# aurelienpierreeng/ansel

Hardware: AMD Instinct MI355X
Metric: MPix/s full export pixelpipe (100 MP raw); % MI355X HBM roofline (higher is better)
Workload: dtype f32

## Files before the change

### ansel_amd/csrc/denoiseprofile.hip

```cpp
#define ANSEL_MATH_DEFAULT_TABS tabs_lds
#include "hip_common.h"
#include "pipe_fused.h"
#include "rgb_chain_kernel.h"
#include "devmath.h"
#include "nlmeans_core_params.h"

#include <math.h>
#include <utility>

using namespace ansel;

namespace
{

#define BANDS DT_HIP_DENOISEPROFILE_BANDS
#define P_FULCRUM 0.05f

__host__ __device__ __forceinline__ float max_first(const float a, const float b) { return a > b ? a : b; }
__host__ __device__ __forceinline__ float min_first(const float a, const float b) { return a < b ? a : b; }
__device__ __forceinline__ int clampi(const int v, const int lo, const int hi) { return v < lo ? lo : (v > hi ? hi : v); }

struct dn_setup
{
  int max_scale;
// ... 248 lines not shown
  const float k0 = fmaf(x, 1056964608.0f - 1065353216.0f, 1065353216.0f);
  return __int_as_float(k0 >= 8388608.0f ? (int)k0 : 0);
}

__device__ __forceinline__ float mexp2_of_clamped(const float arg)
{
  const float k0 = fmaf(arg, 1056964608.0f - 1065353216.0f, 1065353216.0f);
  int k;
  asm("v_cvt_i32_f32 %0, %1" : "=v"(k) : "v"(k0));
  k = min(k, 0x3f800000);
  return __int_as_float(k >= 0x800000 ? k : 0);
}

__device__ __forceinline__ int walk_row(const int b, const int height, const int mult)
{
  if(height <= mult) return b < height ? b : -1;
  const int per_pass = (height + mult - 1) / mult;
  const int row = (b % per_pass) * mult + b / per_pass;
  return row < height ? row : -1;
}

__device__ __forceinline__ double wave_sum_halving(double v)
{
#pragma unroll
  for(int off = 32; off >= 1; off >>= 1) v += __shfl_down(v, off, 64);
  return v;
}

#ifdef ANSEL_HIP_MEASURING
__global__ __launch_bounds__(256) void dn_decompose(const float4 *__restrict__ in, float4 *__restrict__ coarse,
                                                    float4 *__restrict__ detail, double *__restrict__ partial,
                                                    const int width, const int height, const int mult,
                                                    const float inv_sigma2, const int nseg, const int in_row0,
                                                    const int in_rows)
{
  __shared__ double runs[4][4];
  const int bx = xcd_col();
  if(bx >= nseg) return;
  const int row = walk_row(blockIdx.y, height, mult);
  if(row < 0) return;
  const int col = bx * 256 + threadIdx.x;
  double sq[4] = { 0.0, 0.0, 0.0, 0.0 };
  if(col < width)
  {
    const float4 px = in[(size_t)(row + in_row0) * width + col];
    float sum[4] = { 0.f, 0.f, 0.f, 0.f }, wgt = 0.f;
#pragma unroll
    for(int jj = 0; jj < 5; jj++)
    {
      const size_t y = (size_t)clampi(row + in_row0 + mult * (jj - 2), 0, in_rows - 1) * width;
      const float fj = jj == 0 || jj == 4 ? 0.0625f : (jj == 2 ? 0.375f : 0.25f);
#pragma unroll
      for(int ii = 0; ii < 5; ii++)
      {
        const int x = clampi(col + mult * (ii - 2), 0, width - 1);
        const float fi = ii == 0 || ii == 4 ? 0.0625f : (ii == 2 ? 0.375f : 0.25f);
        const float4 p2 = in[y + x];
        const float dx = px.x - p2.x, dy = px.y - p2.y, dz = px.z - p2.z;
        const float dot = (dx * dx + dy * dy + dz * dz) * inv_sigma2;
        const float arg = dot * 0.02f - 9.0f;
        const float wp = mexp2_of_clamped(arg);
        const float w = (fi * fj) * wp;
        wgt += w;
        sum[0] += w * p2.x;
        sum[1] += w * p2.y;
        sum[2] += w * p2.z;
        sum[3] += w * p2.w;
      }
    }
    float c4[4], d4[4];
    const float pin[4] = { px.x, px.y, px.z, px.w };
#pragma unroll
    for(int c = 0; c < 4; c++)
    {
      c4[c] = sum[c] / wgt;
      d4[c] = pin[c] - c4[c];
      sq[c] = (double)(d4[c] * d4[c]);
    }
    const size_t o = (size_t)row * width + col;
    coarse[o] = make_float4(c4[0], c4[1], c4[2], c4[3]);
    if(detail) detail[o] = make_float4(d4[0], d4[1], d4[2], d4[3]);
  }
  const int wave = threadIdx.x >> 6, lane = threadIdx.x & 63;
#pragma unroll
  for(int c = 0; c < 4; c++)
  {
    const double s = wave_sum_halving(sq[c]);
    if(lane == 0) runs[wave][c] = s;
  }
  __syncthreads();
  if(threadIdx.x < 4)
  {
    const int c = threadIdx.x;
    const double seg = ((runs[0][c] + runs[1][c]) + runs[2][c]) + runs[3][c];
    partial[4 * ((size_t)row * nseg + bx) + c] = seg;
  }
}
#endif

#define DN_RING 6
__device__ __forceinline__ float dn_photometric(const float4 px, const float4 p2, const float inv_sigma2)
{
  const float dx = px.x - p2.x, dy = px.y - p2.y, dz = px.z - p2.z;
  const float dot = (dx * dx + dy * dy + dz * dz) * inv_sigma2;
  const float arg = dot * 0.02f - 9.0f;
  return mexp2_of_clamped(arg);
}
__device__ __forceinline__ double wave_sum4_halving(const double q0, const double q1, const double q2, const double q3)
{
  union d2
  {
    double d;
    unsigned u[2];
  };
  auto level = [](const double a, const double b, const bool rows16) {
    d2 x, y, rx, ry;
    x.d = a;
    y.d = b;
#pragma unroll
    for(int h = 0; h < 2; h++)
    {
      const auto r = rows16 ? __builtin_amdgcn_permlane16_swap(x.u[h], y.u[h], false, false)
                            : __builtin_amdgcn_permlane32_swap(x.u[h], y.u[h], false, false);
      rx.u[h] = r[0];
      ry.u[h] = r[1];
    }
    return rx.d + ry.d;
  };
  const double s01 = level(q0, q1, false), s23 = level(q2, q3, false);
  d2 t;
  t.d = level(s01, s23, true);
#define DN_ROW_SHL(n)                                                                                     \
  {                                                                                                       \
    d2 o;                                                                                                 \
    o.u[0] = (unsigned)__builtin_amdgcn_update_dpp(0, (int)t.u[0], 0x100 + (n), 0xf, 0xf, true);          \
    o.u[1] = (unsigned)__builtin_amdgcn_update_dpp(0, (int)t.u[1], 0x100 + (n), 0xf, 0xf, true);          \
    t.d = t.d + o.d;                                                                                      \
  }
  DN_ROW_SHL(8)
  DN_ROW_SHL(4)
  DN_ROW_SHL(2)
  DN_ROW_SHL(1)
#undef DN_ROW_SHL
  return t.d;
}

struct dn_strip_kernargs
{
  const float4 *in;
  float4 *coarse, *detail;
  double *partial;
  int width, height, mult_arg;
  float inv_sigma2;
  int nseg, in_row0, in_rows, strip, strips_per_class;
  vst_args fa;
  unsigned *alpha_flag;
  int flag_sense;
};
template <bool PRE, int MULT, bool ALPHA0> constexpr int dn_strip_waves()
{
  if(PRE && MULT == 0) return 6;
  const int lds = DN_RING * (256 + 4 * (MULT ? MULT : 1)) * (ALPHA0 ? 12 : 16);
  const int wgs = (160 * 1024) / lds;
  return wgs >= 8 ? 8 : (wgs < 1 ? 1 : wgs);
}
template <bool PRE, int MULT, bool ALPHA0, bool P3 = false>
__global__ __launch_bounds__(256) __attribute__((amdgpu_waves_per_eu(dn_strip_waves<PRE, MULT, ALPHA0>(), 8))) void dn_decompose_strip(const float4 *__restrict__ in, float4 *__restrict__ coarse,
                                                          float4 *__restrict__ detail, double *__restrict__ partial,
                                                          const int width, const int height, const int mult_arg,
                                                          const float inv_sigma2, const int nseg, const int in_row0,
                                                          const int in_rows, const int strip, const int strips_per_class,
                                                          const vst_args fa_by_value, unsigned *__restrict__ alpha_flag, const int flag_sense)
{
  const vst_args &fa = kernarg_at<vst_args>((int)offsetof(dn_strip_kernargs, fa));
  (void)fa_by_value;
  if(PRE) ansel_math::stage_default_tables(threadIdx.x);
  if(flag_sense == 1 && *alpha_flag) return;
  if(flag_sense == 2 && !*alpha_flag) return;
  unsigned alpha_bits = 0;
  const int mult = MULT ? MULT : mult_arg;
  constexpr bool LATE2 = PRE && MULT == 1;
  const bool have_t3 = PRE && fa.vst == 2;
  const float t3_of_zero = have_t3 ? dn_vst_y0u0v0_alpha(0.0f, fa) : 0.0f;
#define DN_FETCH(p) (PRE ? dn_precondition_pixel((p), fa, t3_of_zero, have_t3) : (p))
  static_assert(!P3 || ALPHA0, "three-float planes are the ALPHA0 launches'");
  auto in_at = [&](const size_t i) -> float4 {
    if(P3 && !PRE)
    {
      const float *const p3 = reinterpret_cast<const float *>(in) + 3 * i;
      return make_float4(p3[0], p3[1], p3[2], 0.0f);
    }
    return in[i];
  };
  auto plane_put = [&](float4 *const plane, const size_t i, const float v0, const float v1, const float v2, const float v3) {
    if(P3)
    {
      float *const p3 = reinterpret_cast<float *>(plane) + 3 * i;
      p3[0] = v0;
      p3[1] = v1;
      p3[2] = v2;
    }
    else
      plane[i] = make_float4(v0, v1, v2, v3);
  };
  __shared__ double runs[2][4][4];
  const int bx = blockIdx.x;
  const int cls = blockIdx.y / strips_per_class, k0 = (blockIdx.y - cls * strips_per_class) * strip;
  const int n_cls = (height - cls + mult - 1) / mult;
  if(k0 >= n_cls) return;
  const int nrows = min(strip, n_cls - k0);
  const int r_first = cls + k0 * mult;
  const int tw = 256 + 4 * mult;
  extern __shared__ float4 ring[];
  float *const ringf = reinterpret_cast<float *>(ring);
  auto ring_put = [&](const int slot, const int c, const float4 v) {
    if(ALPHA0)
    {
      ringf[(slot * 3 + 0) * tw + c] = v.x;
      ringf[(slot * 3 + 1) * tw + c] = v.y;
      ringf[(slot * 3 + 2) * tw + c] = v.z;
    }
    else
      ring[slot * tw + c] = v;
  };
  auto ring_get = [&](const int slot, const int c) -> float4 {
    if(ALPHA0) return make_float4(ringf[(slot * 3 + 0) * tw + c], ringf[(slot * 3 + 1) * tw + c], ringf[(slot * 3 + 2) * tw + c], 0.0f);
    return ring[slot * tw + c];
  };
  const int tid = threadIdx.x, wave = tid >> 6, lane = tid & 63;
  const int col = bx * 256 + tid;
  const int ecol0 = clampi(bx * 256 - 2 * mult + tid, 0, width - 1), ecol1 = clampi(bx * 256 - 2 * mult + tid + 256, 0, width - 1);
  const bool second = tid + 256 < tw;
#define DN_IN_ROW(q) ((size_t)clampi(r_first + ((q) - 2) * mult + in_row0, 0, in_rows - 1) * width)
#pragma unroll
  for(int q = 0; q < 4; q++)
  {
    const size_t y = DN_IN_ROW(q);
    ring_put(q, tid, DN_FETCH(in_at(y + ecol0)));
    if(second) ring_put(q, tid + 256, DN_FETCH(in_at(y + ecol1)));
  }
  float4 n0, n1 = make_float4(0.f, 0.f, 0.f, 0.f);
  {
    const size_t y = DN_IN_ROW(4);
    n0 = in_at(y + ecol0);
    if(!LATE2 && second) n1 = in_at(y + ecol1);
  }
  int s0 = 0;
  float up1 = 0.f, up2 = 0.f, up2_next = 0.f;
  __syncthreads();
  {
    const float4 c0 = ring_get(2, tid + 2 * mult), c1 = ring_get(3, tid + 2 * mult);
    const float4 a0 = ring_get(0, tid + 2 * mult), a1 = ring_get(1, tid + 2 * mult);
    up2 = dn_photometric(c0, a0, inv_sigma2);
    up1 = dn_photometric(c0, a1, inv_sigma2);
    up2_next = dn_photometric(c1, a1, inv_sigma2);
  }
  for(int k = 0; k < nrows; k++)
  {
    {
      const int sl = s0 + 4 >= DN_RING ? s0 + 4 - DN_RING : s0 + 4;
      ring_put(sl, tid, DN_FETCH(n0));
      if(LATE2) { if(second) ring_put(sl, tid + 256, DN_FETCH(in_at(DN_IN_ROW(k + 4) + ecol1))); }
      else if(second) ring_put(sl, tid + 256, DN_FETCH(n1));
    }
    __syncthreads();
    if(k > 0 && tid < 4)
    {
      const int c = tid, pr = (k - 1) & 1;
      const double seg = ((runs[pr][0][c] + runs[pr][1][c]) + runs[pr][2][c]) + runs[pr][3][c];
      partial[4 * ((size_t)(r_first + (k - 1) * mult) * nseg + bx) + c] = seg;
    }
    if(k + 1 < nrows)
    {
      const size_t y = DN_IN_ROW(k + 5);
      n0 = in_at(y + ecol0);
      if(!LATE2 && second) n1 = in_at(y + ecol1);
    }
    const int row = r_first + k * mult;
    double sq[4] = { 0.0, 0.0, 0.0, 0.0 };
    if(col < width)
    {
      const int sc = s0 + 2 >= DN_RING ? s0 + 2 - DN_RING : s0 + 2;
      const float4 px = ring_get(sc, tid + 2 * mult);
      float sum[4] = { 0.f, 0.f, 0.f, 0.f }, wgt = 0.f, down1 = 0.f, down2 = 0.f;
#pragma unroll
      for(int jj = 0; jj < 5; jj++)
      {
        const int sl = s0 + jj >= DN_RING ? s0 + jj - DN_RING : s0 + jj;
        const float fj = jj == 0 || jj == 4 ? 0.0625f : (jj == 2 ? 0.375f : 0.25f);
        float4 tap[5];
#pragma unroll
        for(int ii = 0; ii < 5; ii++) tap[ii] = ring_get(sl, tid + ii * mult);
#pragma unroll
        for(int ii = 0; ii < 5; ii++)
        {
          const float fi = ii == 0 || ii == 4 ? 0.0625f : (ii == 2 ? 0.375f : 0.25f);
          const float4 p2 = tap[ii];
          float wp;
          if(ii == 2 && jj == 0) wp = up2;
          else if(ii == 2 && jj == 1) wp = up1;
          else wp = dn_photometric(px, p2, inv_sigma2);
          if(ii == 2 && jj == 3) down1 = wp;
          if(ii == 2 && jj == 4) down2 = wp;
          const float w = (fi * fj) * wp;
          wgt += w;
          sum[0] += w * p2.x;
          sum[1] += w * p2.y;
          sum[2] += w * p2.z;
          if(!ALPHA0) sum[3] += w * p2.w;
        }
        asm volatile("" : "+v"(wgt), "+v"(sum[0]), "+v"(sum[1]), "+v"(sum[2]), "+v"(sum[3]) : : "memory");
      }
      up1 = down1;
      up2 = up2_next;
      up2_next = down2;
      float c4[4], d4[4];
      const float pin[4] = { px.x, px.y, px.z, px.w };
#pragma unroll
      for(int c = 0; c < 4; c++)
      {
        if(ALPHA0 && c == 3)
        {
          c4[3] = __builtin_amdgcn_ballot_w64(!(wgt > 0.0f)) == 0ull ? 0.0f : 0.0f / wgt;
          alpha_bits |= __float_as_uint(c4[3]);
        }
        else
          c4[c] = sum[c] / wgt;
        d4[c] = pin[c] - c4[c];
        sq[c] = (double)(d4[c] * d4[c]);
      }
      const size_t o = (size_t)row * width + col;
      plane_put(coarse, o, c4[0], c4[1], c4[2], c4[3]);
      if(detail) plane_put(detail, o, d4[0], d4[1], d4[2], d4[3]);
    }
    {
      const double s = wave_sum4_halving(sq[0], sq[1], sq[2], sq[3]);
      if((lane & 15) == 0) runs[k & 1][wave][((lane >> 5) & 1) | ((lane >> 3) & 2)] = s;
    }
    s0 = s0 + 1 == DN_RING ? 0 : s0 + 1;
  }
#undef DN_IN_ROW
#undef DN_FETCH
  __syncthreads();
  if(tid < 4)
  {
    const int c = tid, pr = (nrows - 1) & 1;
    const double seg = ((runs[pr][0][c] + runs[pr][1][c]) + runs[pr][2][c]) + runs[pr][3][c];
    partial[4 * ((size_t)(r_first + (nrows - 1) * mult) * nseg + bx) + c] = seg;
  }
  if(ALPHA0 && alpha_flag && __builtin_amdgcn_ballot_w64(alpha_bits != 0) != 0ull && lane == 0) atomicOr(alpha_flag, 1u);
}

static void launch_decompose(hipStream_t st, const float4 *in, float4 *coarse, float4 *detail, double *partial, const int width,
                             const int height, const int mult, const float inv_sigma2, const int nseg, const int in_row0,
                             const int in_rows, const vst_args *pre = nullptr, unsigned *alpha_flag = nullptr, const int mode = 0)
{
#ifdef ANSEL_HIP_MEASURING
  static const bool per_row = getenv("ANSEL_HIP_DN_PER_ROW") != nullptr;
  if(per_row && !pre)
  {
    const int rows = (height <= mult) ? height : ((height + mult - 1) / mult) * mult;
    dn_decompose<<<dim3(xcd_pad(nseg), rows), 256, 0, st>>>(in, coarse, detail, partial, width, height, mult, inv_sigma2, nseg,
                                                            in_row0, in_rows);
    return;
  }
#endif
  const int classes = height < mult ? height : mult, per_class = (height + mult - 1) / mult;
  const int strip = strip_rows(nseg, classes, per_class);
  const int strips_per_class = (per_class + strip - 1) / strip;
  const dim3 grid(nseg, classes * strips_per_class);
  size_t lds = (size_t)DN_RING * (256 + 4 * mult) * sizeof(float);
#ifdef ANSEL_HIP_MEASURING
  static const char *const pad_env = measuring_env("ANSEL_HIP_DN_LDS_PAD");
  const size_t lds_pad = pad_env ? (size_t)atoi(pad_env) : 0;
#else
  const size_t lds_pad = 0;
#endif
#define DN_LDS(A0_) (lds * ((A0_) ? 3 : 4) + lds_pad)
  vst_args none;
  memset(&none, 0, sizeof(none));
#define DN_LAUNCH_(PRE_, M_, A0_, FA_, SENSE_)                                                                                          \
  dn_decompose_strip<PRE_, M_, A0_><<<grid, 256, DN_LDS(A0_), st>>>(in, coarse, detail, partial, width, height, mult, inv_sigma2, nseg, in_row0, \
                                                            in_rows, strip, strips_per_class, FA_, alpha_flag, SENSE_)
#define DN_LAUNCH(PRE_, M_, FA_)                  \
  do                                              \
  {                                               \
    if(mode == 1)                                 \
      dn_decompose_strip<PRE_, M_, true, true><<<grid, 256, DN_LDS(true), st>>>(in, coarse, detail, partial, width, height, mult, inv_sigma2, nseg, in_row0, \
                                                            in_rows, strip, strips_per_class, FA_, alpha_flag, 0); \
    else if(mode == 2)                            \
      DN_LAUNCH_(PRE_, M_, false, FA_, 2);        \
    else if(alpha_flag && (PRE_))                 \
      DN_LAUNCH_(PRE_, M_, true, FA_, 0);         \
    else if(alpha_flag)                           \
    {                                             \
      DN_LAUNCH_(PRE_, M_, true, FA_, 1);         \
      DN_LAUNCH_(PRE_, M_, false, FA_, 2);        \
    }                                             \
    else                                          \
      DN_LAUNCH_(PRE_, M_, false, FA_, 0);        \
  } while(0)
  if(pre)
  {
    if(mult == 1) DN_LAUNCH(true, 1, *pre);
    else DN_LAUNCH(true, 0, *pre);
  }
  else
    switch(mult)
    {
      case 1: DN_LAUNCH(false, 1, none); break;
      case 2: DN_LAUNCH(false, 2, none); break;
      case 4: DN_LAUNCH(false, 4, none); break;
      case 8: DN_LAUNCH(false, 8, none); break;
      case 16: DN_LAUNCH(false, 16, none); break;
      case 32: DN_LAUNCH(false, 32, none); break;
      case 64: DN_LAUNCH(false, 64, none); break;
      default: DN_LAUNCH(false, 0, none); break;
    }
#undef DN_LAUNCH
#undef DN_LAUNCH_
#undef DN_LDS
}

struct thr_args
{
  size_t n_partial;
  float n1;
  float sb2;
  float adjt[4];
};

#define THR_GROUPS 16
__global__ __launch_bounds__(64) void dn_band_sums(const double *__restrict__ partial_all, const size_t n_partial,
                                                  double *__restrict__ acc_all )
{
  const double *const partial = partial_all + (size_t)blockIdx.y * n_partial * 4;
  double *const acc = acc_all + (size_t)blockIdx.y * 4 * 1024;
  const int t = blockIdx.x * 64 + threadIdx.x;
  double s[4] = { 0.0, 0.0, 0.0, 0.0 };
  typedef double d4 __attribute__((ext_vector_type(4)));
  const d4 *const p4 = (const d4 *)partial;
  size_t k = t;
  for(; k + 7 * 1024 < n_partial; k += 8 * 1024)
  {
    d4 v[8];
#pragma unroll
    for(int u = 0; u < 8; u++) v[u] = p4[k + (size_t)u * 1024];
#pragma unroll
    for(int u = 0; u < 8; u++)
    {
      s[0] += v[u].x;
      s[1] += v[u].y;
      s[2] += v[u].z;
      s[3] += v[u].w;
    }
  }
  for(; k < n_partial; k += 1024)
  {
    const d4 v = p4[k];
    s[0] += v.x;
    s[1] += v.y;
    s[2] += v.z;
    s[3] += v.w;
  }
#pragma unroll
  for(int c = 0; c < 4; c++) acc[c * 1024 + t] = s[c];
}

struct thr_args_all
{
  thr_args band[BANDS];
};
__global__ __launch_bounds__(1024) void dn_band_threshold(const double *__restrict__ sums_all ,
                                                          const thr_args_all all, float *__restrict__ thrs_all)
{
  __shared__ double acc[4][1024];
  const double *const sums = sums_all + (size_t)blockIdx.x * 4 * 1024;
  const thr_args &a = all.band[blockIdx.x];
  float *const thrs = thrs_all + 4 * blockIdx.x;
  const int t = threadIdx.x;
#pragma unroll
  for(int c = 0; c < 4; c++) acc[c][t] = sums[c * 1024 + t];
  __syncthreads();
  for(int off = 512; off >= 1; off >>= 1)
  {
    if(t < off)
    {
#pragma unroll
      for(int c = 0; c < 4; c++) acc[c][t] += acc[c][t + off];
    }
    __syncthreads();
  }
  if(t < 4)
  {
    const float sum_y2 = (float)acc[t][0];
    const float std_x = t < 3 ? sqrtf(max_first(1e-6f, sum_y2 / a.n1 - a.sb2)) : 1.0f;
    thrs[t] = a.adjt[t] * a.sb2 / std_x;
  }
}


bool invert3(const float in[3][4], float out[3][4])
{
  const float A = in[1][1] * in[2][2] - in[1][2] * in[2][1];
  const float B = -in[1][0] * in[2][2] + in[1][2] * in[2][0];
  const float C = in[1][0] * in[2][1] - in[1][1] * in[2][0];
  const float D = -in[0][1] * in[2][2] + in[0][2] * in[2][1];
  const float E = in[0][0] * in[2][2] - in[0][2] * in[2][0];
  const float F = -in[0][0] * in[2][1] + in[0][1] * in[2][0];
  const float G = in[0][1] * in[1][2] - in[0][2] * in[1][1];
  const float H = -in[0][0] * in[1][2] + in[0][2] * in[1][0];
  const float I = in[0][0] * in[1][1] - in[0][1] * in[1][0];
  const float det = in[0][0] * A + in[0][1] * B + in[0][2] * C;
  if(det == 0.0f) return false;
  const float r = 1.0f / det;
  out[0][0] = r * A; out[0][1] = r * D; out[0][2] = r * G; out[0][3] = 0.0f;
  out[1][0] = r * B; out[1][1] = r * E; out[1][2] = r * H; out[1][3] = 0.0f;
  out[2][0] = r * C; out[2][1] = r * F; out[2][2] = r * I; out[2][3] = 0.0f;
  return true;
}

void setup(const dt_hip_piece_t *piece, const dt_hip_denoiseprofile_data_t *d, dn_setup &s, const bool nlm)
{
  memset(&s, 0, sizeof(s));
  const float in_scale = fminf((float)piece->roi_in.scale, 1.0f);
  const float big = (float)(piece->roi_in.height > piece->roi_in.width ? piece->roi_in.height : piece->roi_in.width);
  const float supp0 = min_first((float)(2 * (2u << (BANDS - 1)) + 1), big * 0.2f);
  const float i0 = log2f((supp0 - 1.0f) * .5f);
  int max_scale = 0;
  for(; max_scale < BANDS; max_scale++)
  {
    const float supp = (float)(2 * (2u << max_scale) + 1);
    const float supp_in = supp * (1.0f / in_scale);
    const float i_in = log2f((supp_in - 1) * .5f) - 1.0f;
    const float t = 1.0f - (i_in + .5f) / i0;
    if(t < 0.0f) break;
  }
  s.max_scale = max_scale;

  const float weights[4] = { nlm ? 1.0f : 2.0f, 1.0f, nlm ? 1.0f : 2.0f, 0.0f };
  const float wb_mean = (d->wb_coeffs[0] + d->wb_coeffs[1] + d->wb_coeffs[2]) / 3.0f;
  float *wb = s.wb;
// ... 216 lines not shown
    synth_args none;
    memset(&none, 0, sizeof(none));
    dn_finish<<<pixel_grid(npix_out), 256, 0, st>>>((float4 *)dev_out, nullptr, npix_out, ia, none);
  }
  return check_launch("dn_finish");
}

int wavelets_runnable(const dt_hip_piece_t *piece, const dn_setup &s)
{
  const int w = piece->roi_in.width, h = piece->roi_in.height;
  if(s.max_scale < 1)
  {
    set_last_error("denoiseprofile: frame too small for a single wavelet band");
    return -1;
  }
  const int max_mult = 1 << (s.max_scale - 1);
  if(w < 2 * max_mult || h < 2 * max_mult) return 0;
  if(w < 4 * max_mult)
  {
    set_last_error("denoiseprofile: %d columns is less than 4x the coarsest dilation %d", w, max_mult);
    return -1;
  }
  return 1;
}

}

namespace ansel
{

struct dn_band_job_t
{
  int devid, w, frame_h, max_scale, row0, rows;
  dt_hip_denoiseprofile_data_t d;
  dn_setup s;
  dev_buf_t cur;
  int cur_top, cur_bottom;
  dev_buf_t det[BANDS];
  dev_buf_t sums;
  dev_buf_t local;
  dev_buf_t thrs;
  int next_scale;
  bool sums_requested;
};

void denoiseprofile_band_abort(dn_band_job_t *j)
{
  delete j;
}

int denoiseprofile_halo_rows(const dt_hip_piece_t *piece, const dt_hip_denoiseprofile_data_t *d)
{
  if(DT_HIP_DENOISEPROFILE_IS_NLMEANS(d->mode)) return nlmeans_core_halo_rows(piece->roi_in.height, nlm_params_of(piece, d));
  dn_setup s;
  setup(piece, d, s, false);
  if(wavelets_runnable(piece, s) != 1) return -1;
  return 2;
}

static int clip_halo(const int h, const int avail) { return h < avail ? h : avail; }

int denoiseprofile_band_begin(int devid, const dt_hip_piece_t *piece, const dt_hip_denoiseprofile_data_t *d,
                              const band_view_t *band, const int buf_rows, dt_hip_mem_t dev_in, dt_hip_mem_t dev_out,
                              dn_band_job_t **job)
{
  *job = nullptr;
  if(!valid_device(devid) || !piece || !d || !band || !dev_in || buf_rows <= 0) return DT_HIP_INVALID_ARG;
  if(piece->channels != 4 || !(piece->roi_in.scale > 0.0)) return DT_HIP_INVALID_ARG;
  if(DT_HIP_DENOISEPROFILE_IS_NLMEANS(d->mode)) return denoise_nlmeans(devid, piece, d, band, buf_rows, dev_in, dev_out);
  if(!DT_HIP_DENOISEPROFILE_IS_WAVELETS(d->mode)) return DT_HIP_INVALID_ARG;
  dn_band_job_t *j = new dn_band_job_t();
  j->devid = devid;
  j->w = piece->roi_in.width;
  j->frame_h = band->frame_h;
  j->row0 = band->row0;
  j->rows = band->row1 - band->row0;
  j->d = *d;
  setup(piece, d, j->s, false);
  if(wavelets_runnable(piece, j->s) != 1)
  {
    delete j;
    return DT_HIP_INVALID_ARG;
  }
  j->max_scale = j->s.max_scale;
  const int w = j->w, nseg = (w + 255) / 256;
  const size_t npix = (size_t)w * buf_rows;
  const size_t n_frame = (size_t)band->frame_h * nseg;
  const size_t sums_bytes = (size_t)j->max_scale * n_frame * 4 * sizeof(double);
  j->cur_top = band->row0 - band->buf_row0;
  j->cur_bottom = buf_rows - j->cur_top - j->rows;
  bool ok = (bool)(j->cur = dev_buf_t::alloc(devid, npix * sizeof(float4)));
  ok &= (bool)(j->sums = dev_buf_t::alloc(devid, sums_bytes));
  ok &= (bool)(j->local = dev_buf_t::alloc(devid, (size_t)j->rows * nseg * 4 * sizeof(double)));
  ok &= (bool)(j->thrs = dev_buf_t::alloc(devid, BANDS * 4 * sizeof(float)));
  if(!ok || j->cur_bottom < 0)
  {
    denoiseprofile_band_abort(j);
    return DT_HIP_SYSMEM_ALLOCATION;
  }
  hipStream_t st = stream_of(devid);
  if(hipMemsetAsync(j->sums.ptr(), 0, sums_bytes, st) != hipSuccess)
  {
    denoiseprofile_band_abort(j);
    return DT_HIP_DEFAULT_ERROR;
  }
  {
    vst_args fa;
    forward_args(j->s, fa);
    launch_scope ls(devid, "dn_precondition");
    dn_precondition<<<pixel_grid(npix), 256, 0, st>>>((const float4 *)dev_in, j->cur.as<float4>(), npix, fa);
  }
  const int err = check_launch("dn_precondition");
  if(err != DT_HIP_SUCCESS)
  {
    denoiseprofile_band_abort(j);
    return err;
  }
  *job = j;
  return DT_HIP_SUCCESS;
}

int denoiseprofile_band_step(dn_band_job_t *j, dt_hip_mem_t *halo_buf, int *halo_rows, double **sums, size_t *sum_count)
{
  *halo_buf = nullptr;
  *halo_rows = 0;
  *sums = nullptr;
  *sum_count = 0;
  const int devid = j->devid, w = j->w, nseg = (w + 255) / 256;
  const size_t n_frame = (size_t)j->frame_h * nseg;
  if(j->next_scale >= j->max_scale)
  {
    if(j->sums_requested) return 0;
    j->sums_requested = true;
    *sums = j->sums.as<double>();
    *sum_count = (size_t)j->max_scale * n_frame * 4;
    return 2;
  }
  hipStream_t st = stream_of(devid);
  const int scale = j->next_scale, mult = 1 << scale;
  const bool last = scale + 1 == j->max_scale;
  const int h_next = last ? 0 : 2 * (2 << scale);
  const int top = clip_halo(h_next, j->row0), bottom = clip_halo(h_next, j->frame_h - j->row0 - j->rows);
  dev_buf_t coarse = dev_buf_t::alloc(devid, (size_t)(top + j->rows + bottom) * w * sizeof(float4));
  j->det[scale] = dev_buf_t::alloc(devid, (size_t)j->rows * w * sizeof(float4));
  if(!coarse || !j->det[scale])
  {
    denoiseprofile_band_abort(j);
    return DT_HIP_SYSMEM_ALLOCATION;
  }
  const float varf = sqrtf(2.0f + 2.0f * 4.0f * 4.0f + 6.0f * 6.0f) / 16.0f;
  const float sigma_band = powf(varf, scale) * 1.0f;
  {
    launch_scope ls(devid, "dn_decompose");
    launch_decompose(st, j->cur.as<float4>(), coarse.as<float4>() + (size_t)top * w, j->det[scale].as<float4>(), j->local.as<double>(), w, j->rows, mult,
                     1.0f / (sigma_band * sigma_band), nseg, j->cur_top, j->cur_top + j->rows + j->cur_bottom);
  }
  int err = check_launch("denoiseprofile band decompose");
  if(err == DT_HIP_SUCCESS
     && hipMemcpyAsync(j->sums.as<double>() + ((size_t)scale * n_frame + (size_t)j->row0 * nseg) * 4, j->local.ptr(),
                       (size_t)j->rows * nseg * 4 * sizeof(double), hipMemcpyDeviceToDevice, st) != hipSuccess)
    err = DT_HIP_DEFAULT_ERROR;
  j->cur = std::move(coarse);
  j->cur_top = top;
  j->cur_bottom = bottom;
  j->next_scale++;
  if(err != DT_HIP_SUCCESS)
  {
    denoiseprofile_band_abort(j);
    return err;
  }
  if(!last && (top || bottom))
  {
    *halo_buf = j->cur.ptr();
    *halo_rows = h_next;
    return 1;
  }
  return denoiseprofile_band_step(j, halo_buf, halo_rows, sums, sum_count);
}

int denoiseprofile_band_finish(dn_band_job_t *j, dt_hip_mem_t dev_out)
{
  if(!j || !dev_out) return DT_HIP_INVALID_ARG;
  const int devid = j->devid, nseg = (j->w + 255) / 256;
  const size_t npix = (size_t)j->w * j->rows, n_frame = (size_t)j->frame_h * nseg;
  hipStream_t st = stream_of(devid);
  float4 *out = (float4 *)dev_out;
  int err = DT_HIP_SUCCESS;
  synth_args sy;
  memset(&sy, 0, sizeof(sy));
  sy.nbands = j->max_scale;
  sy.thrs = j->thrs.as<float>();
  const dev_buf_t accs_buf = dev_buf_t::alloc(devid, (size_t)BANDS * 4 * 1024 * sizeof(double));
  double *const accs = accs_buf.as<double>();
  if(!accs) err = DT_HIP_SYSMEM_ALLOCATION;
  thr_args_all all;
  memset(&all, 0, sizeof(all));
  for(int scale = 0; scale < j->max_scale; scale++)
  {
    all.band[scale].n_partial = n_frame;
    threshold_args(&j->d, scale, j->max_scale, (size_t)j->w * j->frame_h, all.band[scale]);
    sy.detail[scale] = j->det[scale].as<float4>();
  }
  if(err == DT_HIP_SUCCESS)
  {
    launch_scope ls(devid, "dn_band_threshold");
    dn_band_sums<<<dim3(THR_GROUPS, j->max_scale), 64, 0, st>>>(j->sums.as<double>(), n_frame, accs);
    dn_band_threshold<<<j->max_scale, 1024, 0, st>>>(accs, all, j->thrs.as<float>());
    err = check_launch("denoiseprofile band threshold");
  }
  if(err == DT_HIP_SUCCESS)
  {
    vst_args ia;
    inverse_args(j->s, ia);
    launch_scope ls(devid, "dn_finish");
    dn_finish<<<pixel_grid(npix), 256, 0, st>>>(out, j->cur.as<float4>() + (size_t)j->cur_top * j->w, npix, ia, sy);
    err = check_launch("dn_finish");
  }
  denoiseprofile_band_abort(j);
  return err;
}

}

extern "C" {

static int denoiseprofile_run(int devid, const dt_hip_piece_t *piece, const dt_hip_denoiseprofile_data_t *d, dt_hip_mem_t dev_in,
                              dt_hip_mem_t dev_out, const rgb_group_t *chain)
{
  if(!valid_device(devid) || !piece || !d || !dev_in || !dev_out) return DT_HIP_INVALID_ARG;
  if(!DT_HIP_DENOISEPROFILE_IS_WAVELETS(d->mode) && !DT_HIP_DENOISEPROFILE_IS_NLMEANS(d->mode))
  {
    set_last_error("denoiseprofile: mode %d is not implemented on device (wavelets and non-local means are)", d->mode);
    return DT_HIP_INVALID_ARG;
  }
  if(piece->channels != 4 || !(piece->roi_in.scale > 0.0)) return DT_HIP_INVALID_ARG;
  const int w = piece->roi_in.width, h = piece->roi_in.height;
  if(w <= 0 || h <= 0) return DT_HIP_SUCCESS;
  const size_t npix = (size_t)w * h, plane = npix * sizeof(float4);
  if(DT_HIP_DENOISEPROFILE_IS_NLMEANS(d->mode))
    return chain ? DT_HIP_INVALID_ARG : denoise_nlmeans(devid, piece, d, nullptr, h, dev_in, dev_out);
  chain_args ca;
  int cm_kind = CM_NONE, fm = FM_NONE;
  if(chain)
  {
    if(chain->pre_lab || chain->to_u16 || chain->width != w || chain->height != h) return DT_HIP_INVALID_ARG;
    if(rgb_group_fill_args(*chain, ca, cm_kind, fm) != DT_HIP_SUCCESS || fm != FM_NONE) return DT_HIP_INVALID_ARG;
  }
  dn_setup s;
  setup(piece, d, s, false);
  const int runnable = wavelets_runnable(piece, s);
  if(runnable < 0) return DT_HIP_INVALID_ARG;
  hipStream_t st = stream_of(devid);
  if(!runnable) return chain ? DT_HIP_INVALID_ARG : dt_hip_enqueue_copy_buffer_to_buffer(devid, dev_in, dev_out, 0, 0, plane);
  const int nseg = (w + 255) / 256;
  const size_t n_partial = (size_t)h * nseg;
  const dev_buf_t partial_buf = dev_buf_t::alloc(devid, (size_t)BANDS * n_partial * 4 * sizeof(double));
  const dev_buf_t thrs_buf = dev_buf_t::alloc(devid, BANDS * 4 * sizeof(float));
  const dev_buf_t accs_buf = dev_buf_t::alloc(devid, (size_t)BANDS * 4 * 1024 * sizeof(double));
  double *const partial = partial_buf.as<double>(), *const accs = accs_buf.as<double>();
  float *const thrs = thrs_buf.as<float>();
  int err = (partial && thrs && accs) ? DT_HIP_SUCCESS : DT_HIP_SYSMEM_ALLOCATION;
  synth_args sy;
  memset(&sy, 0, sizeof(sy));
  sy.nbands = s.max_scale;
  sy.thrs = thrs;
  dev_buf_t coarse_buf[BANDS];
  float4 *coarse[BANDS] = { nullptr };
  const dev_buf_t det0_buf = dev_buf_t::alloc(devid, plane);
  float4 *const det0 = det0_buf.as<float4>();
  if(!det0) err = DT_HIP_SYSMEM_ALLOCATION;
  for(int k = 0; k < s.max_scale && err == DT_HIP_SUCCESS; k++)
  {
    coarse[k] = (coarse_buf[k] = dev_buf_t::alloc(devid, plane)).as<float4>();
    if(!coarse[k]) err = DT_HIP_SYSMEM_ALLOCATION;
    sy.detail[k] = k == 0 ? det0 : coarse[k];
  }
  sy.coarse0 = coarse[0];
  float4 *out = (float4 *)dev_out;
  vst_args fa;
  forward_args(s, fa);
  const float4 *b1 = (const float4 *)dev_in;
  dev_buf_t alpha_buf;
  unsigned *alpha_flag = nullptr;
  if(err == DT_HIP_SUCCESS && s.vst == 2)
  {
    alpha_flag = (alpha_buf = dev_buf_t::alloc(devid, sizeof(unsigned))).as<unsigned>();
    if(!alpha_flag) err = DT_HIP_SYSMEM_ALLOCATION;
    else if(hipMemsetAsync(alpha_flag, 0, sizeof(unsigned), st) != hipSuccess) err = DT_HIP_DEFAULT_ERROR;
  }
  const int sequences = alpha_flag ? 2 : 1;
  for(int seq = 0; seq < sequences && err == DT_HIP_SUCCESS; seq++)
  {
    b1 = (const float4 *)dev_in;
    for(int scale = 0; scale < s.max_scale && err == DT_HIP_SUCCESS; scale++)
    {
      const int mult = 1 << scale;
      const float varf = sqrtf(2.0f + 2.0f * 4.0f * 4.0f + 6.0f * 6.0f) / 16.0f;
      const float sigma_band = powf(varf, scale) * 1.0f;
      {
        launch_scope ls(devid, "dn_decompose");
        launch_decompose(st, b1, coarse[scale], scale == 0 ? det0 : nullptr, partial + (size_t)scale * n_partial * 4, w, h, mult,
                         1.0f / (sigma_band * sigma_band), nseg, 0, h, scale == 0 ? &fa : nullptr, alpha_flag, alpha_flag ? seq + 1 : 0);
      }
      err = check_launch("denoiseprofile band");
      b1 = coarse[scale];
    }
  }
  if(err == DT_HIP_SUCCESS)
  {
    thr_args_all all;
    memset(&all, 0, sizeof(all));
    for(int scale = 0; scale < s.max_scale; scale++)
    {
      all.band[scale].n_partial = n_partial;
      threshold_args(d, scale, s.max_scale, npix, all.band[scale]);
    }
    launch_scope ls(devid, "dn_band_threshold");
    dn_band_sums<<<dim3(THR_GROUPS, s.max_scale), 64, 0, st>>>(partial, n_partial, accs);
    dn_band_threshold<<<s.max_scale, 1024, 0, st>>>(accs, all, thrs);
    err = check_launch("denoiseprofile thresholds");
  }
  if(err == DT_HIP_SUCCESS)
  {
    vst_args ia;
    inverse_args(s, ia);
    const unsigned grid = pixel_grid(npix);
    for(int seq = 0; seq < sequences; seq++)
    {
      launch_scope ls(devid, chain ? "dn_finish_chain" : "dn_finish");
      if(alpha_flag)
      {
        sy.planes3 = seq == 0;
        sy.gate = alpha_flag;
        sy.gate_sense = seq + 1;
      }
      if(!chain) dn_finish<<<grid, 256, 0, st>>>(out, b1, npix, ia, sy);
      else
        switch(cm_kind)
        {
          case CM_NONE: dn_finish_chain<CM_NONE><<<grid, 256, 0, st>>>(out, b1, npix, ia, sy, ca); break;
          case 0: dn_finish_chain<0><<<grid, 256, 0, st>>>(out, b1, npix, ia, sy, ca); break;
          case 1: dn_finish_chain<1><<<grid, 256, 0, st>>>(out, b1, npix, ia, sy, ca); break;
          case 2: dn_finish_chain<2><<<grid, 256, 0, st>>>(out, b1, npix, ia, sy, ca); break;
          case 3: dn_finish_chain<3><<<grid, 256, 0, st>>>(out, b1, npix, ia, sy, ca); break;
          default: dn_finish_chain<4><<<grid, 256, 0, st>>>(out, b1, npix, ia, sy, ca); break;
        }
    }
    err = check_launch("dn_finish");
  }
  return err;
}

int dt_hip_iop_denoiseprofile_process(int devid, const dt_hip_piece_t *piece, const dt_hip_denoiseprofile_data_t *d,
                                      dt_hip_mem_t dev_in, dt_hip_mem_t dev_out)
{
  return denoiseprofile_run(devid, piece, d, dev_in, dev_out, nullptr);
}
}

namespace ansel
{
int denoiseprofile_process_chain(int devid, const dt_hip_piece_t *piece, const dt_hip_denoiseprofile_data_t *d,
                                 dt_hip_mem_t dev_in, dt_hip_mem_t dev_out, const rgb_group_t *chain)
{
  if(!chain) return DT_HIP_INVALID_ARG;
  return denoiseprofile_run(devid, piece, d, dev_in, dev_out, chain);
}
}

extern "C" {


void dt_hip_iop_denoiseprofile_tiling(const dt_hip_piece_t *piece, const dt_hip_denoiseprofile_data_t *d,
                                      dt_hip_tiling_t *tiling)
{
  memset(tiling, 0, sizeof(*tiling));
  tiling->maxbuf = tiling->maxbuf_cl = 1.0f;
  tiling->xalign = tiling->yalign = 1;
  if(DT_HIP_DENOISEPROFILE_IS_NLMEANS(d->mode))
  {
    const float scale = fminf(fminf((float)piece->roi_in.scale, 2.0f), 1.0f);
    const int P = (int)ceilf(d->radius * scale), K = (int)ceilf(d->nbhood * scale);
    const int K_scattered = (int)ceilf(d->scattering * (K * K * K + 7.0 * K * sqrt((double)K)) / 6.0) + K;
    tiling->factor = 2.0f + 0.25f;
    tiling->factor_cl = 3.0f;
    tiling->overlap = (unsigned)(P + K_scattered);
  }
  else
  {
    dn_setup s;
    setup(piece, d, s, false);
    tiling->factor = 5.0f;
    tiling->factor_cl = 3.0f + (float)s.max_scale + 1.0f / 64.0f;
    tiling->overlap = 1u << s.max_scale;
  }
}

}
```

### ansel_amd/csrc/diffuse.hip

```cpp
#include "hip_common.h"

#include <type_traits>
#include "devmath.h"
#include "ieee_inrange.h"
#include "px_colorspaces.h"

#include <math.h>
#include <cstdlib>

namespace ansel
{
int bspline_launch_decompose(int devid, hipStream_t s, const float4 *in, float4 *hf, float4 *lf, int w, int h, int mult,
                             const unsigned *gate = nullptr);
int bspline_launch_decompose3(int devid, hipStream_t s, const void *in, bool in4, float *lf, int w, int h, int mult, unsigned *alpha_flag);
#ifdef ANSEL_HIP_MEASURING
int bspline_launch_decompose2(int devid, hipStream_t s, const float4 *in, float4 *low1, float4 *low2, int w, int h, int mult);
#endif
}
using namespace ansel;

namespace
{

#define DIFFUSE_MAX_SCALES 10
// ... 250 lines not shown
      H4[3 * ii + jj] = hf[rows[ii] + cols[jj]];
      L4[3 * ii + jj] = lf[rows[ii] + cols[jj]];
    }
  const int tw = 256 + 2 * a.mult;
  const int tx = threadIdx.x;
  float4 energy = make_float4(0.f, 0.f, 0.f, 0.f);
  if(SHARED)
  {
#pragma unroll
    for(int ii = 0; ii < 3; ii++)
    {
      const float4 h = H4[3 * ii + 1], l = L4[3 * ii + 1];
      r2s[ii * tw + tx + a.mult] = make_float4(ratio2(h.x, l.x), ratio2(h.y, l.y), ratio2(h.z, l.z), ratio2(h.w, l.w));
    }
    if(tx < a.mult)
    {
#pragma unroll
      for(int ii = 0; ii < 3; ii++)
      {
        const float4 h = H4[3 * ii], l = L4[3 * ii];
        r2s[ii * tw + tx] = make_float4(ratio2(h.x, l.x), ratio2(h.y, l.y), ratio2(h.z, l.z), ratio2(h.w, l.w));
      }
    }
    if(tx >= 256 - a.mult)
    {
#pragma unroll
      for(int ii = 0; ii < 3; ii++)
      {
        const float4 h = H4[3 * ii + 2], l = L4[3 * ii + 2];
        r2s[ii * tw + tx + 2 * a.mult] = make_float4(ratio2(h.x, l.x), ratio2(h.y, l.y), ratio2(h.z, l.z), ratio2(h.w, l.w));
      }
    }
    __syncthreads();
    if(col >= a.width) return;
#pragma unroll
    for(int ii = 0; ii < 3; ii++)
    {
#pragma unroll
      for(int jj = 0; jj < 3; jj++)
      {
        const float4 r = r2s[ii * tw + tx + jj * a.mult];
        energy.x += r.x;
        energy.y += r.y;
        energy.z += r.z;
        energy.w += r.w;
      }
      asm volatile("" : "+v"(energy.x), "+v"(energy.y), "+v"(energy.z), "+v"(energy.w) : : "memory");
    }
  }
  else
  {
    if(col >= a.width) return;
#pragma unroll
    for(int k = 0; k < 9; k++)
    {
      energy.x += ratio2(H4[k].x, L4[k].x);
      energy.y += ratio2(H4[k].y, L4[k].y);
      energy.z += ratio2(H4[k].z, L4[k].z);
      energy.w += ratio2(H4[k].w, L4[k].w);
    }
  }
  if(mask && !mask[(size_t)row * a.width + col])
  {
    const size_t c = (size_t)row * a.width + col;
    const float4 h = H4[4], l = L4[4];
    const float4 o = make_float4(max_zero(h.x + l.x), max_zero(h.y + l.y), max_zero(h.z + l.z), max_zero(h.w + l.w));
    if(final_pass) nt_store(out + c, o);
    else out[c] = o;
    return;
  }
  float H[9], L[9];
  float4 o;
#pragma unroll
  for(int k = 0; k < 9; k++) { H[k] = H4[k].x; L[k] = L4[k].x; }
  o.x = pde_channel(H, L, energy.x, a);
#pragma unroll
  for(int k = 0; k < 9; k++) { H[k] = H4[k].y; L[k] = L4[k].y; }
  o.y = pde_channel(H, L, energy.y, a);
#pragma unroll
  for(int k = 0; k < 9; k++) { H[k] = H4[k].z; L[k] = L4[k].z; }
  o.z = pde_channel(H, L, energy.z, a);
  if(alpha_is_blank(H4, L4))
    o.w = 0.0f;
  else
  {
#pragma unroll
    for(int k = 0; k < 9; k++) { H[k] = H4[k].w; L[k] = L4[k].w; }
    o.w = pde_channel(H, L, energy.w, a);
  }
  const size_t idx = rows[1] + col;
  if(final_pass) nt_store(out + idx, o);
  else out[idx] = o;
}

#define PDE_RING 4
#define PDE_DMA_MAX_MULT 16
#if defined(__HIP_DEVICE_COMPILE__) && !defined(__gfx950__)
#error "pde_dma_planes(): LDS-DMA of 16 bytes per lane and its hazard padding are written for gfx950 only"
#endif
template <int NPL>
__device__ __forceinline__ void pde_dma_planes(const float4 *const p0, const float4 *const p1, const float4 *const p2, const unsigned voff,
                                               const unsigned d0, const unsigned d1, const unsigned d2)
{
  unsigned keep;
  if constexpr(NPL == 3)
    asm volatile("s_waitcnt lgkmcnt(0)\n\ts_nop 4\n\ts_mov_b32 %0, m0\n\t"
                 "s_mov_b32 m0, %5\n\ts_nop 0\n\tglobal_load_lds_dwordx4 %1, %2\n\t"
                 "s_mov_b32 m0, %6\n\ts_nop 0\n\tglobal_load_lds_dwordx4 %1, %3\n\t"
                 "s_mov_b32 m0, %7\n\ts_nop 0\n\tglobal_load_lds_dwordx4 %1, %4\n\t"
                 "s_mov_b32 m0, %0"
                 : "=&s"(keep)
                 : "v"(voff), "s"(p0), "s"(p1), "s"(p2), "s"(d0), "s"(d1), "s"(d2)
                 : "memory");
  else
    asm volatile("s_waitcnt lgkmcnt(0)\n\ts_nop 4\n\ts_mov_b32 %0, m0\n\t"
                 "s_mov_b32 m0, %4\n\ts_nop 0\n\tglobal_load_lds_dwordx4 %1, %2\n\t"
                 "s_mov_b32 m0, %5\n\ts_nop 0\n\tglobal_load_lds_dwordx4 %1, %3\n\t"
                 "s_mov_b32 m0, %0"
                 : "=&s"(keep)
                 : "v"(voff), "s"(p0), "s"(p2), "s"(d0), "s"(d2)
                 : "memory");
}
template <bool H0_4>
__device__ __forceinline__ void pde_dma_planes3(const void *const p0, const void *const p1, const void *const p2, const unsigned voff0,
                                                const unsigned voff, const unsigned d0, const unsigned d1, const unsigned d2)
{
  unsigned keep;
  if constexpr(H0_4)
    asm volatile("s_waitcnt lgkmcnt(0)\n\ts_nop 4\n\ts_mov_b32 %0, m0\n\t"
                 "s_mov_b32 m0, %6\n\ts_nop 0\n\tglobal_load_lds_dwordx4 %1, %3\n\t"
                 "s_mov_b32 m0, %7\n\ts_nop 0\n\tglobal_load_lds_dwordx3 %2, %4\n\t"
                 "s_mov_b32 m0, %8\n\ts_nop 0\n\tglobal_load_lds_dwordx3 %2, %5\n\t"
                 "s_mov_b32 m0, %0"
                 : "=&s"(keep)
                 : "v"(voff0), "v"(voff), "s"(p0), "s"(p1), "s"(p2), "s"(d0), "s"(d1), "s"(d2)
                 : "memory");
  else
    asm volatile("s_waitcnt lgkmcnt(0)\n\ts_nop 4\n\ts_mov_b32 %0, m0\n\t"
                 "s_mov_b32 m0, %5\n\ts_nop 0\n\tglobal_load_lds_dwordx3 %1, %2\n\t"
                 "s_mov_b32 m0, %6\n\ts_nop 0\n\tglobal_load_lds_dwordx3 %1, %3\n\t"
                 "s_mov_b32 m0, %7\n\ts_nop 0\n\tglobal_load_lds_dwordx3 %1, %4\n\t"
                 "s_mov_b32 m0, %0"
                 : "=&s"(keep)
                 : "v"(voff), "s"(p0), "s"(p1), "s"(p2), "s"(d0), "s"(d1), "s"(d2)
                 : "memory");
}
struct pde_px3
{
  float x, y, z;
};
template <bool HSUB, int MODE, bool DMA, int L3>
__device__ __forceinline__ void pde_strip_body(const float4 *__restrict__ hf, const float4 *__restrict__ hsub,
                                               const float4 *__restrict__ lf, float4 *__restrict__ out, const pde_args &a,
                                               const int final_pass, const unsigned char *__restrict__ mask, const int strip,
                                               const int strips_per_class)
{
  static_assert(L3 == 0 || (HSUB && DMA), "three-float planes: the low-pass chain's LDS-DMA form only");
  if(a.gate && ((*a.gate != 0u) == (a.gate_sense == 1))) return;
  extern __shared__ float4 r2s[];
  pde_px3 *const r2s3 = reinterpret_cast<pde_px3 *>(r2s);
  const int mult = a.mult;
  const int cls = blockIdx.y / strips_per_class, k0s = (blockIdx.y - cls * strips_per_class) * strip;
  const int n_cls = (a.height - cls + mult - 1) / mult;
  if(k0s >= n_cls) return;
  const int nrows = (strip < n_cls - k0s) ? strip : n_cls - k0s;
  const int r_first = cls + k0s * mult;
  const int tx = threadIdx.x, tw = 256 + 2 * mult;
  const int col = (int)blockIdx.x * 256 + tx;
  const bool live = col < a.width;
  const int cols[3] = { clampi(col - mult, 0, a.width - 1), clampi(col, 0, a.width - 1), clampi(col + mult, 0, a.width - 1) };
#define PDE_ROW(v) ((size_t)clampi(r_first + ((v) - 1) * mult, 0, a.height - 1) * a.width)
  float4 Hw[3][3], Lw[3][3];
  constexpr int NPL = HSUB ? 3 : 2;
  const int lane = tx & 63, zw = 64 + 2 * mult;
  float4 *const zone = r2s + PDE_RING * tw + (tx >> 6) * NPL * zw;
  float4 *const zone3 = reinterpret_cast<float4 *>(reinterpret_cast<char *>(r2s) + (size_t)PDE_RING * tw * 12) + (tx >> 6) * 3 * zw;
  using lds_f4_ptr = __attribute__((address_space(3))) float4 *;
  const unsigned zone_lds = !DMA ? 0u : (unsigned)__builtin_amdgcn_readfirstlane((int)(unsigned)(__UINTPTR_TYPE__)(lds_f4_ptr)(
                                           L3 ? zone3 : zone));
  const unsigned off_main = (unsigned)cols[0] * 16u, off_halo = (unsigned)clampi(col - mult + 64, 0, a.width - 1) * 16u;
  auto dma_row = [&](const int v) {
    const size_t y = PDE_ROW(v);
    if constexpr(L3 != 0)
    {
      const unsigned m3 = (unsigned)cols[0] * 12u, h3 = (unsigned)clampi(col - mult + 64, 0, a.width - 1) * 12u;
      const unsigned p0 = (unsigned)zw * 16u, p1 = 2u * p0;
      const void *const b0 = L3 == 2 ? (const void *)(hf + y) : (const void *)((const float *)hf + 3 * y);
      const void *const b1 = (const float *)hsub + 3 * y, *const b2 = (const float *)lf + 3 * y;
      pde_dma_planes3<L3 == 2>(b0, b1, b2, L3 == 2 ? off_main : m3, m3, zone_lds, zone_lds + p0, zone_lds + p1);
      if(lane < 2 * mult)
        pde_dma_planes3<L3 == 2>(b0, b1, b2, L3 == 2 ? off_halo : h3, h3, zone_lds + 1024u, zone_lds + p0 + 1024u, zone_lds + p1 + 1024u);
      return;
    }
    const unsigned pl = (unsigned)zw * 16u;
    pde_dma_planes<NPL>(hf + y, hsub + y, lf + y, off_main, zone_lds, zone_lds + pl, zone_lds + (NPL - 1) * pl);
    if(lane < 2 * mult)
      pde_dma_planes<NPL>(hf + y, hsub + y, lf + y, off_halo, zone_lds + 1024u, zone_lds + pl + 1024u, zone_lds + (NPL - 1) * pl + 1024u);
  };
  struct
  {
    float4 o;
    size_t idx;
    bool have;
  } pending;
  pending.have = false;
  auto store = [&](const size_t i, const float4 o) {
    if(final_pass) nt_store(out + i, o);
    else if constexpr(L3 != 0)
    {
      float *const p3 = (float *)out + 3 * i;
      p3[0] = o.x;
      p3[1] = o.y;
      p3[2] = o.z;
    }
    else out[i] = o;
  };
  auto fetch_row = [&](const int v, auto slot_tag) {
    constexpr int SL = decltype(slot_tag)::value;
    const size_t y = PDE_ROW(v);
    float4 c[3], low[3];
    if constexpr(DMA)
    {
      asm volatile("s_waitcnt vmcnt(0)" : : : "memory");
      if constexpr(L3 != 0)
      {
#pragma unroll
        for(int jj = 0; jj < 3; jj++)
        {
          const int x = lane + jj * mult;
          const float4 v0 = zone3[x], v1 = zone3[zw + x], v2 = zone3[2 * zw + x];
          c[jj] = make_float4(v0.x, v0.y, v0.z, 0.0f);
          low[jj] = make_float4(v1.x, v1.y, v1.z, 0.0f);
          Lw[SL][jj] = make_float4(v2.x, v2.y, v2.z, 0.0f);
        }
      }
      else
#pragma unroll
      for(int jj = 0; jj < 3; jj++)
      {
        c[jj] = zone[lane + jj * mult];
        if(HSUB) low[jj] = zone[zw + lane + jj * mult];
        Lw[SL][jj] = zone[(NPL - 1) * zw + lane + jj * mult];
      }
    }
    else if(PDE_OFF(a, 2) && v >= 2)
    {
#pragma unroll
      for(int jj = 0; jj < 3; jj++)
      {
        c[jj] = Hw[SL][jj];
        low[jj] = make_float4(0.f, 0.f, 0.f, 0.f);
      }
    }
    else
    {
#pragma unroll
      for(int jj = 0; jj < 3; jj++)
      {
        c[jj] = hf[y + cols[jj]];
        if(HSUB) low[jj] = hsub[y + cols[jj]];
        Lw[SL][jj] = lf[y + cols[jj]];
      }
    }
    __builtin_amdgcn_sched_barrier(0);
#pragma unroll
    for(int jj = 0; jj < 3; jj++)
      Hw[SL][jj] = HSUB ? make_float4(c[jj].x - low[jj].x, c[jj].y - low[jj].y, c[jj].z - low[jj].z, c[jj].w - low[jj].w) : c[jj];
    float4 *const ring = r2s + (v % PDE_RING) * tw;
    auto ratios = [&](const float4 h, const float4 l) {
      const bool blank = a.wskip && __builtin_amdgcn_ballot_w64((__float_as_uint(h.w) | __float_as_uint(l.w)) != 0) == 0ull;
      return ratio2_rgb(h, l, blank ? 0.0f : ratio2(h.w, l.w), PDE_APPROX(a));
    };
    if(PDE_OFF(a, 4)) return;
    if constexpr(L3 != 0)
    {
      pde_px3 *const ring3 = r2s3 + (v % PDE_RING) * tw;
      auto put = [&](const int x, const float4 h, const float4 l) {
        const float4 r = ratio2_rgb(h, l, 0.0f, PDE_APPROX(a));
        ring3[x] = { r.x, r.y, r.z };
      };
      put(tx + mult, Hw[SL][1], Lw[SL][1]);
      if(tx < mult) put(tx, Hw[SL][0], Lw[SL][0]);
      if(tx >= 256 - mult) put(tx + 2 * mult, Hw[SL][2], Lw[SL][2]);
      return;
    }
    ring[tx + mult] = ratios(Hw[SL][1], Lw[SL][1]);
    if(tx < mult) ring[tx] = ratios(Hw[SL][0], Lw[SL][0]);
    if(tx >= 256 - mult) ring[tx + 2 * mult] = ratios(Hw[SL][2], Lw[SL][2]);
  };
  auto row_step = [&](auto t_tag, const int kk) {
    constexpr int T = decltype(t_tag)::value, S0 = T, S1 = (T + 1) % 3, S2 = (T + 2) % 3;
    constexpr bool WIDE_READS = MODE >= 0 && !(((MODE % 3) | ((MODE / 9) % 3)) && (((MODE / 3) % 3) | ((MODE / 27) % 3)));
    fetch_row(kk + 2, std::integral_constant<int, S2>());
    if constexpr(DMA)
    {
      if(pending.have)
      {
        store(pending.idx, pending.o);
        pending.have = false;
      }
      if(kk + 1 < nrows) dma_row(kk + 3);
    }
    if(!PDE_OFF(a, 1)) __syncthreads();
    if(!live) return;
    const float4 H4[9] = { Hw[S0][0], Hw[S0][1], Hw[S0][2], Hw[S1][0], Hw[S1][1], Hw[S1][2], Hw[S2][0], Hw[S2][1], Hw[S2][2] };
    const float4 L4[9] = { Lw[S0][0], Lw[S0][1], Lw[S0][2], Lw[S1][0], Lw[S1][1], Lw[S1][2], Lw[S2][0], Lw[S2][1], Lw[S2][2] };
    const int row = r_first + kk * mult;
    const bool blank = L3 != 0 || alpha_is_blank(H4, L4);
    __builtin_amdgcn_sched_barrier(0);
    if(pending.have && !PDE_OFF(a, 8))
    {
      store(pending.idx, pending.o);
      pending.have = false;
    }
    __builtin_amdgcn_sched_barrier(0);
    float4 energy = make_float4(0.f, 0.f, 0.f, 0.f);
    if(PDE_OFF(a, 4)) energy = make_float4(0.5f, 0.5f, 0.5f, 0.5f);
    else if constexpr(L3 != 0)
#pragma unroll
    for(int ii = 0; ii < 3; ii++)
    {
      const pde_px3 *const ring = r2s3 + ((kk + ii) % PDE_RING) * tw + tx;
#pragma unroll
      for(int jj = 0; jj < 3; jj++)
      {
        const pde_px3 r = ring[jj * mult];
        energy.x += r.x;
        energy.y += r.y;
        energy.z += r.z;
      }
      if(!WIDE_READS || ii >= 1) asm volatile("" : "+v"(energy.x), "+v"(energy.y), "+v"(energy.z) : : "memory");
    }
    else
#pragma unroll
    for(int ii = 0; ii < 3; ii++)
    {
      const float4 *const ring = r2s + ((kk + ii) % PDE_RING) * tw + tx;
#pragma unroll
      for(int jj = 0; jj < 3; jj++)
      {
        const float4 r = ring[jj * mult];
        energy.x += r.x;
        energy.y += r.y;
        energy.z += r.z;
        if(!(blank && a.wskip)) energy.w += r.w;
      }
      if(!WIDE_READS || ii >= 1) asm volatile("" : "+v"(energy.x), "+v"(energy.y), "+v"(energy.z), "+v"(energy.w) : : "memory");
    }
    const size_t idx = (size_t)row * a.width + col;
    float4 o;
    if(L3 == 0 && mask && !mask[idx])
    {
      const float4 h = H4[4], l = L4[4];
      o = make_float4(max_zero(h.x + l.x), max_zero(h.y + l.y), max_zero(h.z + l.z), max_zero(h.w + l.w));
    }
    else if(PDE_OFF(a, 16))
      o = make_float4(H4[4].x + energy.x, L4[4].y + energy.y, H4[0].z + energy.z, L4[8].w);
    else
    {
      float H[9], L[9];
#pragma unroll
      for(int k = 0; k < 9; k++) { H[k] = H4[k].x; L[k] = L4[k].x; }
      o.x = pde_channel<MODE>(H, L, energy.x, a);
#pragma unroll
      for(int k = 0; k < 9; k++) { H[k] = H4[k].y; L[k] = L4[k].y; }
      o.y = pde_channel<MODE>(H, L, energy.y, a);
#pragma unroll
      for(int k = 0; k < 9; k++) { H[k] = H4[k].z; L[k] = L4[k].z; }
      o.z = pde_channel<MODE>(H, L, energy.z, a);
      if(blank)
        o.w = 0.0f;
      else
      {
#pragma unroll
        for(int k = 0; k < 9; k++) { H[k] = H4[k].w; L[k] = L4[k].w; }
        o.w = pde_channel<MODE>(H, L, energy.w, a);
      }
    }
    if(a.post_lab) o = px_rgb_to_lab(o, a.post_m);
    pending.o = o;
    pending.idx = idx;
    pending.have = true;
  };
  if constexpr(DMA) dma_row(0);
  fetch_row(0, std::integral_constant<int, 0>());
  if constexpr(DMA) dma_row(1);
  fetch_row(1, std::integral_constant<int, 1>());
  if constexpr(DMA) dma_row(2);
  for(int kk = 0; kk < nrows; kk += 3)
  {
    row_step(std::integral_constant<int, 0>(), kk);
    if(kk + 1 < nrows) row_step(std::integral_constant<int, 1>(), kk + 1);
    if(kk + 2 < nrows) row_step(std::integral_constant<int, 2>(), kk + 2);
  }
  if constexpr(DMA) asm volatile("s_waitcnt vmcnt(0)" : : : "memory");
  if(pending.have) store(pending.idx, pending.o);
#undef PDE_ROW
}

template <bool HSUB, int MODE, bool DMA = false>
__global__ __launch_bounds__(256, 3) void diffuse_pde_strip(const float4 *__restrict__ hf, const float4 *__restrict__ hsub,
                                                         const float4 *__restrict__ lf,
                                                         float4 *__restrict__ out, const pde_args a, const int final_pass,
                                                         const unsigned char *__restrict__ mask, const int strip,
                                                         const int strips_per_class)
{
  pde_strip_body<HSUB, MODE, DMA, 0>(hf, hsub, lf, out, a, final_pass, mask, strip, strips_per_class);
}
template <int MODE, bool H0_4>
__global__ __launch_bounds__(256, 3) void diffuse_pde_strip3(const float4 *__restrict__ hf, const float4 *__restrict__ hsub,
                                                          const float4 *__restrict__ lf, float4 *__restrict__ out, const pde_args a,
                                                          const int final_pass, const int strip, const int strips_per_class)
{
  pde_strip_body<true, MODE, true, H0_4 ? 2 : 1>(hf, hsub, lf, out, a, final_pass, nullptr, strip, strips_per_class);
}

__device__ __forceinline__ uint32_t splitmix32(const uint64_t seed)
{
  uint64_t result = (seed ^ (seed >> 33)) * 0x62a9d9ed799705f5ull;
  result = (result ^ (result >> 28)) * 0xcb24d0a5c88c35b3ull;
  return (uint32_t)(result >> 32);
}

__device__ __forceinline__ float xoshiro128plus(uint32_t state[4])
{
  const uint32_t result = state[0] + state[3];
  const uint32_t t = state[1] << 9;
  state[2] ^= state[0];
  state[3] ^= state[1];
  state[1] ^= state[2];
  state[0] ^= state[3];
  state[2] ^= t;
  state[3] = (state[3] << 11) | (state[3] >> 21);
  return (float)(result >> 8) * 0x1.0p-24f;
}

__device__ __forceinline__ float gaussian_noise(const float mu, const float sigma, const bool flip, uint32_t state[4])
{
  const float x1 = xoshiro128plus(state);
  const float u1 = x1 > 1.17549435e-38f ? x1 : 1.17549435e-38f;
  const float u2 = xoshiro128plus(state);
  const float angle = (float)(6.283185307179586 * (double)u2);
  const float radius = sqrtf(-2.0f * ansel_math::logf_exact(u1));
  const float noise = flip ? radius * ansel_math::cosf_exact(angle) : radius * ansel_math::sinf_exact(angle);
  return noise * sigma + mu;
}

__global__ __launch_bounds__(256) void diffuse_inpaint(const float4 *__restrict__ in, float4 *__restrict__ out,
                                                       unsigned char *__restrict__ mask, const float threshold,
                                                       const size_t npixels, const size_t width, const size_t first_pixel)
{
  const size_t p = (size_t)blockIdx.x * blockDim.x + threadIdx.x;
  if(p >= npixels) return;
  const float4 v = in[p];
  const bool m = v.x > threshold || v.y > threshold || v.z > threshold;
  mask[p] = m ? 1 : 0;
  float4 o = v;
  if(m)
  {
    const size_t k = 4 * (p + first_pixel);
    const uint32_t i = (uint32_t)(k / width);
    const uint32_t j = (uint32_t)(k - i);
    uint32_t state[4] = { splitmix32((uint32_t)(j + 1)), splitmix32((uint64_t)(uint32_t)(j + 1) * (uint32_t)(i + 3)),
                          splitmix32(1337), splitmix32(666) };
    xoshiro128plus(state);
    xoshiro128plus(state);
    xoshiro128plus(state);
    xoshiro128plus(state);
    const bool flip = (i % 2) || (j % 2);
    o.x = fabsf(gaussian_noise(v.x, v.x, flip, state));
    o.y = fabsf(gaussian_noise(v.y, v.y, flip, state));
    o.z = fabsf(gaussian_noise(v.z, v.z, flip, state));
    o.w = fabsf(gaussian_noise(v.w, v.w, flip, state));
  }
  out[p] = o;
}

inline float sqf(const float x) { return x * x; }

float sigma_at_step(const float sigma, const unsigned s)
{
  float acc = sigma;
  for(unsigned k = 1; k <= s; k++) acc = sqrtf(sqf(acc) + sqf(exp2f((float)k) * sigma));
  return acc;
}

unsigned steps_to_sigma(const float sigma_filter, const float sigma_final)
{
  unsigned s = 0;
  float radius = sigma_filter;
  while(radius < sigma_final)
  {
    ++s;
    radius = sqrtf(sqf(radius) + sqf((float)(1 << s) * sigma_filter));
  }
  return s + 1;
}

int scales_of(const dt_hip_piece_t *piece, const dt_hip_diffuse_data_t *d)
{
  const float zoom = (float)(d->iscale / piece->roi_in.scale);
  const float final_radius = (float)(d->radius + d->radius_center) * 2.0f / zoom;
  const int s = (int)steps_to_sigma(BSPLINE_SIGMA, final_radius);
  return s < 1 ? 1 : (s > DIFFUSE_MAX_SCALES ? DIFFUSE_MAX_SCALES : s);
}

}

namespace ansel
{
int diffuse_halo_rows(const dt_hip_piece_t *piece, const dt_hip_diffuse_data_t *d)
{
  if(!(d->iscale > 0.0f) || !(piece->roi_in.scale > 0.0)) return -1;
  const int scales = scales_of(piece, d);
  const int it_req = (int)ceilf((float)d->iterations);
  const int iterations = it_req > 1 ? it_req : 1;
  return iterations * 3 * ((1 << scales) - 1);
}
}

extern "C" {

int dt_hip_iop_diffuse_process(int devid, const dt_hip_piece_t *piece, const dt_hip_diffuse_data_t *d,
                               dt_hip_mem_t dev_in, dt_hip_mem_t dev_out)
{
  return diffuse_process_rows(devid, piece, d, 0, dev_in, dev_out);
}

}

namespace ansel
{
static void *g_diffuse_probe = nullptr;

static int diffuse_run(int devid, const dt_hip_piece_t *piece, const dt_hip_diffuse_data_t *d, int first_row, dt_hip_mem_t dev_in,
                       dt_hip_mem_t dev_out, const dt_hip_lab_data_t *post_lab);
int diffuse_process_rows(int devid, const dt_hip_piece_t *piece, const dt_hip_diffuse_data_t *d, int first_row,
                         dt_hip_mem_t dev_in, dt_hip_mem_t dev_out)
{
  return diffuse_run(devid, piece, d, first_row, dev_in, dev_out, nullptr);
}
int diffuse_process_post_lab(int devid, const dt_hip_piece_t *piece, const dt_hip_diffuse_data_t *d, dt_hip_mem_t dev_in,
                             dt_hip_mem_t dev_out, const dt_hip_lab_data_t *lab)
{
  if(!lab || measuring_env("ANSEL_HIP_PDE_PER_ROW")) return DT_HIP_INVALID_ARG;
  return diffuse_run(devid, piece, d, 0, dev_in, dev_out, lab);
}

struct diffuse_planes_t
{
  dev_buf_t hf[DIFFUSE_MAX_SCALES], lf[2], tmp[2];
  dev_buf_t mask;
  dev_buf_t inpainted;
  dev_buf_t alpha_flag;
};

struct diffuse_job_t
{
  int devid;
  hipStream_t st;
  const dt_hip_diffuse_data_t *d;
  const dt_hip_lab_data_t *post_lab;
  int w, h, scales, iterations;
  float zoom;
  bool lf_chain;
  bool per_row, no_dma;
  diffuse_planes_t p;
};

static int diffuse_alloc_planes(diffuse_job_t &j, const bool in_place, const bool three)
{
  diffuse_planes_t &p = j.p;
  const size_t plane = (size_t)j.w * j.h * sizeof(float4);
  bool ok = true;
  for(int s = 0; s < j.scales; s++) ok &= (bool)(p.hf[s] = dev_buf_t::alloc(j.devid, plane));
  for(int k = 0; k < ((j.lf_chain && !in_place) ? 1 : 2); k++) ok &= (bool)(p.lf[k] = dev_buf_t::alloc(j.devid, plane));
  for(int k = 0; k < 2 && k < j.iterations - 1; k++) ok &= (bool)(p.tmp[k] = dev_buf_t::alloc(j.devid, plane));
  if(ok && three) ok &= (bool)(p.alpha_flag = dev_buf_t::alloc(j.devid, sizeof(unsigned)));
  if(ok && j.d->threshold > 0.0f)
  {
    p.mask = dev_buf_t::alloc(j.devid, (size_t)j.w * j.h);
    if(!p.tmp[1]) p.tmp[1] = dev_buf_t::alloc(j.devid, plane);
    p.inpainted = dev_buf_t::borrow(p.tmp[1].base());
    ok = p.mask && p.inpainted;
  }
  return ok ? DT_HIP_SUCCESS : DT_HIP_SYSMEM_ALLOCATION;
}

static void pde_args_of_call(pde_args &a, const int w, const int h, const dt_hip_diffuse_data_t *d)
{
  memset(&a, 0, sizeof(a));
  a.width = w;
  a.height = h;
  a.wskip = measuring_env("ANSEL_HIP_PDE_NO_WSKIP") ? 0 : 1;
  const char *const approx_env = measuring_env("ANSEL_HIP_PDE_APPROX_DIV");
  a.approx_div = approx_env && atoi(approx_env) != 0;
  const char *const off_env = measuring_env("ANSEL_HIP_PDE_OFF");
  a.off = off_env ? atoi(off_env) : 0;
  const float user_aniso[4] = { d->anisotropy_first, d->anisotropy_second, d->anisotropy_third, d->anisotropy_fourth };
  for(int k = 0; k < 4; k++)
  {
    a.anisotropy[k] = sqf(user_aniso[k]);
    a.kind[k] = user_aniso[k] == 0.0f ? 0 : (user_aniso[k] > 0.0f ? 1 : 2);
  }
  a.same02 = a.kind[0] == a.kind[2] && a.anisotropy[0] == a.anisotropy[2];
  a.same13 = a.kind[1] == a.kind[3] && a.anisotropy[1] == a.anisotropy[3];
  a.variance_threshold = powf(10.0f, d->variance_threshold);
}

static void pde_args_of_scale(pde_args &a, const diffuse_job_t &j, const int s, const bool last_pass)
{
  const dt_hip_diffuse_data_t *const d = j.d;
  const float regularization = powf(10.0f, d->regularization) - 1.0f;
  const float speed[4] = { d->first, d->second, d->third, d->fourth };
  const float real_radius = sigma_at_step(BSPLINE_SIGMA, (unsigned)s) * j.zoom;
  a.regularization = regularization / 9.0f * sqf(real_radius);
  const float norm = expf(-sqf(real_radius - (float)d->radius_center) / sqf((float)d->radius));
  for(int k = 0; k < 4; k++) a.abcd[k] = speed[k] * PDE_KAPPA * norm;
  a.strength = d->sharpness * norm + 1.0f;
  a.mult = 1 << s;
  a.post_lab = 0;
  if(j.post_lab && last_pass)
  {
    a.post_lab = 1;
    memcpy(a.post_m, j.post_lab->matrix, sizeof(a.post_m));
  }
}

typedef void (*pde_strip_fn)(const float4 *, const float4 *, const float4 *, float4 *, pde_args, int, const unsigned char *, int, int);
typedef void (*pde_strip3_fn)(const float4 *, const float4 *, const float4 *, float4 *, pde_args, int, int, int);

template <int MD> static pde_strip_fn pde_strip_forms(const bool chain, const bool dma)
{
  if(dma) return diffuse_pde_strip<true, MD, true>;
  if(chain) return diffuse_pde_strip<true, MD>;
  return diffuse_pde_strip<false, MD>;
}
static pde_strip_fn pde_strip_kernel(const int mode, const bool chain, const bool dma)
{
  switch(mode)
  {
#define PDE_CASE(MD) \
  case MD: return pde_strip_forms<MD>(chain, dma);
    PDE_MODES(PDE_CASE)
#undef PDE_CASE
    default: return pde_strip_forms<-1>(chain, dma);
  }
}
static pde_strip3_fn pde_strip3_kernel(const int mode, const bool h0_4)
{
  if(mode == PDE_MODE_DEBLUR) return h0_4 ? diffuse_pde_strip3<PDE_MODE_DEBLUR, true> : diffuse_pde_strip3<PDE_MODE_DEBLUR, false>;
  return h0_4 ? diffuse_pde_strip3<PDE_MODE_ISOTROPIC, true> : diffuse_pde_strip3<PDE_MODE_ISOTROPIC, false>;
}

static void pde_strip_launch(const diffuse_job_t &j, const pde_args &a, const bool p3, const bool h0_4, const bool chain,
                             const bool dma, const float4 *h0, const float4 *h1, const float4 *cur, float4 *to,
                             const int final_pass)
{
  const int w = j.w, h = j.h;
  const int classes = h < a.mult ? h : a.mult, per_class = (h + a.mult - 1) / a.mult;
  const int gx = (w + 255) / 256;
  int longest = 32;
#ifdef ANSEL_HIP_MEASURING
  static const char *const strip_env = measuring_env("ANSEL_HIP_PDE_STRIP");
  if(strip_env) longest = atoi(strip_env);
#endif
  const int strip = strip_rows(gx, classes, per_class, longest);
  const int spc = (per_class + strip - 1) / strip;
  size_t ring = (size_t)PDE_RING * (256 + 2 * a.mult) * sizeof(float4);
#ifdef ANSEL_HIP_MEASURING
  static const char *const pad_env = measuring_env("ANSEL_HIP_PDE_LDS_PAD");
  if(pad_env) ring += (size_t)atoi(pad_env);
#endif
  static const bool generic = measuring_env("ANSEL_HIP_PDE_GENERIC") != nullptr;
  const int mode = generic ? -1 : pde_mode_of(a);
  const dim3 sgrid(gx, classes * spc);
  if(p3)
  {
    const size_t lds3 = (size_t)PDE_RING * (256 + 2 * a.mult) * 12 + (size_t)4 * 3 * (64 + 2 * a.mult) * 16;
    pde_strip3_kernel(mode, h0_4)<<<sgrid, 256, lds3, j.st>>>(h0, h1, cur, to, a, final_pass, strip, spc);
    return;
  }
  const size_t lds = dma ? ring + (size_t)4 * 3 * (64 + 2 * a.mult) * sizeof(float4) : ring;
  pde_strip_kernel(mode, chain, dma)<<<sgrid, 256, lds, j.st>>>(h0, h1, cur, to, a, final_pass, j.p.mask.as<unsigned char>(), strip, spc);
}

static int diffuse_iteration(const diffuse_job_t &j, pde_args &a, const bool p3, const bool first, const bool last,
                             const float4 *src, float4 *dst)
{
  const int w = j.w, h = j.h, scales = j.scales;
  float4 *hf[DIFFUSE_MAX_SCALES];
  for(int s = 0; s < DIFFUSE_MAX_SCALES; s++) hf[s] = j.p.hf[s].as<float4>();
  float4 *const lf[2] = { j.p.lf[0].as<float4>(), j.p.lf[1].as<float4>() };
  unsigned *const alpha_flag = j.p.alpha_flag.as<unsigned>();
  const unsigned char *const mask = j.p.mask.as<unsigned char>();
  int err = DT_HIP_SUCCESS;
  const float4 *level = src;
  float4 *residual = lf[0];
  const bool chain = j.lf_chain && (const float4 *)dst != src;
  for(int s = 0; s < scales && err == DT_HIP_SUCCESS; s++)
  {
#ifdef ANSEL_HIP_MEASURING
    static const bool pairs = measuring_env("ANSEL_HIP_BSPLINE_PAIRS") != nullptr;
    if(chain && pairs && s + 1 < scales && (s == 0 || s == 2))
    {
      err = bspline_launch_decompose2(j.devid, j.st, level, hf[s], hf[s + 1], w, h, 1 << s);
      s++;
      level = residual = hf[s];
      continue;
    }
#endif
    float4 *low = chain ? hf[s] : lf[s % 2];
    if(p3) err = bspline_launch_decompose3(j.devid, j.st, level, first && s == 0, (float *)low, w, h, 1 << s, alpha_flag);
    else err = bspline_launch_decompose(j.devid, j.st, level, chain ? nullptr : hf[s], low, w, h, 1 << s, alpha_flag);
    level = low;
    residual = low;
  }
  float4 *pp[2] = { residual == lf[1] ? lf[0] : lf[1], residual };
  const float4 *cur = residual;
  int count = 0;
  for(int s = scales - 1; s >= 0 && err == DT_HIP_SUCCESS; s--, count++)
  {
    pde_args_of_scale(a, j, s, s == 0 && last);
    float4 *to = (s == 0) ? dst : (chain ? (count % 2 == 0 ? lf[0] : hf[s + 1]) : pp[count % 2]);
    {
      launch_scope ls(j.devid, "diffuse_pde");
      if(a.mult <= PDE_SHARED_MULT && !j.per_row)
      {
        const float4 *const h0 = chain ? (s == 0 ? src : hf[s - 1]) : hf[s], *const h1 = chain ? hf[s] : nullptr;
        const bool dma = chain && a.mult <= PDE_DMA_MAX_MULT && !j.no_dma;
        pde_strip_launch(j, a, p3, first && s == 0, chain, dma, h0, h1, cur, to, p3 ? (s == 0 && last) : s == 0);
      }
      else
      {
        const int rows = (h <= a.mult) ? h : ((h + a.mult - 1) / a.mult) * a.mult;
        const dim3 grid(xcd_pad((w + 255) / 256), rows);
        if(a.mult <= PDE_SHARED_MULT)
          diffuse_pde<true><<<grid, 256, (size_t)3 * (256 + 2 * a.mult) * sizeof(float4), j.st>>>(hf[s], cur, to, a, s == 0, mask);
        else
          diffuse_pde<false><<<grid, 256, 0, j.st>>>(hf[s], cur, to, a, s == 0, mask);
      }
    }
    err = check_launch("diffuse_pde");
    cur = to;
  }
  return err;
}

static int diffuse_run(int devid, const dt_hip_piece_t *piece, const dt_hip_diffuse_data_t *d, int first_row, dt_hip_mem_t dev_in,
                       dt_hip_mem_t dev_out, const dt_hip_lab_data_t *post_lab)
{
  if(!valid_device(devid) || !piece || !d || !dev_in || !dev_out) return DT_HIP_INVALID_ARG;
  if(piece->channels != 4)
  {
    set_last_error("diffuse: needs a 4-channel float input");
    return DT_HIP_INVALID_ARG;
  }
  const int w = piece->roi_out.width, h = piece->roi_out.height;
  if(w <= 0 || h <= 0) return DT_HIP_SUCCESS;
  if(!(d->iscale > 0.0f) || !(piece->roi_in.scale > 0.0)) return DT_HIP_INVALID_ARG;
  static const bool per_row_pde = measuring_env("ANSEL_HIP_PDE_PER_ROW") != nullptr;
  static const bool hf_planes = measuring_env("ANSEL_HIP_DIFFUSE_HF_PLANES") != nullptr;
  static const bool no_dma = measuring_env("ANSEL_HIP_PDE_NO_DMA") != nullptr;
  const int it_req = (int)ceilf((float)d->iterations);
  diffuse_job_t j;
  j.devid = devid;
  j.st = stream_of(devid);
  j.d = d;
  j.post_lab = post_lab;
  j.w = w, j.h = h;
  j.scales = scales_of(piece, d);
  j.iterations = it_req > 1 ? it_req : 1;
  j.zoom = (float)(d->iscale / piece->roi_in.scale);
  j.lf_chain = !per_row_pde && !hf_planes && (1 << (j.scales - 1)) <= PDE_SHARED_MULT;
  j.per_row = per_row_pde, j.no_dma = no_dma;
  const int iterations = j.iterations;
  pde_args a;
  pde_args_of_call(a, w, h, d);

  const int mode0 = pde_mode_of(a);
  const bool in_place = iterations == 1 && dev_in == dev_out && !(d->threshold > 0.0f);
  const bool three = j.lf_chain && !no_dma && !(d->threshold > 0.0f) && (1 << (j.scales - 1)) <= PDE_DMA_MAX_MULT &&
                     !(iterations == 1 && dev_in == dev_out) && !measuring_env("ANSEL_HIP_PDE_GENERIC") &&
                     (mode0 == PDE_MODE_DEBLUR || mode0 == PDE_MODE_ISOTROPIC);
  int err = diffuse_alloc_planes(j, in_place, three);
  unsigned *const alpha_flag = j.p.alpha_flag.as<unsigned>();
  if(err == DT_HIP_SUCCESS && alpha_flag && hipMemsetAsync(alpha_flag, 0, sizeof(unsigned), j.st) != hipSuccess) err = DT_HIP_DEFAULT_ERROR;
  const float4 *src = (const float4 *)dev_in;
  if(err == DT_HIP_SUCCESS && j.p.mask)
  {
    const size_t np = (size_t)w * h;
    launch_scope ls(devid, "diffuse_inpaint");
    diffuse_inpaint<<<pixel_grid(np), 256, 0, j.st>>>(src, j.p.inpainted.as<float4>(), j.p.mask.as<unsigned char>(), d->threshold, np,
                                                      (size_t)w, (size_t)first_row * w);
    err = check_launch("diffuse_inpaint");
    src = j.p.inpainted.as<float4>();
  }
  for(int seq = alpha_flag ? 0 : 1; seq < 2 && err == DT_HIP_SUCCESS; seq++)
  {
    const bool p3 = seq == 0;
    a.gate = alpha_flag;
    a.gate_sense = p3 ? 1 : 2;
    if(alpha_flag) src = (const float4 *)dev_in;
    for(int it = 0; err == DT_HIP_SUCCESS && it < iterations; it++)
    {
      float4 *dst = (it == iterations - 1) ? (float4 *)dev_out : j.p.tmp[it % 2].as<float4>();
      err = diffuse_iteration(j, a, p3, it == 0, it == iterations - 1, src, dst);
      src = dst;
    }
  }
  if(alpha_flag)
  {
    if(g_diffuse_probe && err == DT_HIP_SUCCESS
       && hipMemcpyAsync(g_diffuse_probe, alpha_flag, sizeof(unsigned), hipMemcpyDeviceToDevice, j.st) != hipSuccess)
      err = DT_HIP_DEFAULT_ERROR;
  }
  else if(g_diffuse_probe && err == DT_HIP_SUCCESS && hipMemsetAsync(g_diffuse_probe, 0xff, sizeof(unsigned), j.st) != hipSuccess)
    err = DT_HIP_DEFAULT_ERROR;
  return err;
}

}

extern "C" {

int dt_hip_test_diffuse_probe(void *sink)
{
  ansel::g_diffuse_probe = sink;
  return DT_HIP_SUCCESS;
}

void dt_hip_iop_diffuse_tiling(const dt_hip_piece_t *piece, const dt_hip_diffuse_data_t *d, dt_hip_tiling_t *tiling)
{
  const int scales = scales_of(piece, d);
  tiling->factor = 6.0625f + scales;
  tiling->factor_cl = 6.0625f + scales;
  tiling->maxbuf = 1.0f;
// ... 9 lines not shown
```

### ansel_amd/csrc/diffuse_bspline.hip

```cpp
#include "hip_common.h"

#include <cstdlib>

using namespace ansel;

namespace
{

__device__ __forceinline__ float max_first(const float a, const float b) { return a > b ? a : b; }
__device__ __forceinline__ int clampi(const int v, const int lo, const int hi) { return v < lo ? lo : (v > hi ? hi : v); }

__device__ __forceinline__ float tap5(const float a, const float b, const float c, const float d, const float e)
{
  const float s = 0.0625f * a + 0.25f * b + 0.375f * c + 0.25f * d + 0.0625f * e;
  return max_first(0.0f, s);
}
__device__ __forceinline__ float4 tap5(const float4 a, const float4 b, const float4 c, const float4 d, const float4 e)
{
  return make_float4(tap5(a.x, b.x, c.x, d.x, e.x), tap5(a.y, b.y, c.y, d.y, e.y), tap5(a.z, b.z, c.z, d.z, e.z),
                     tap5(a.w, b.w, c.w, d.w, e.w));
}

__device__ __forceinline__ int walk_row(const int b, const int height, const int mult)
{
  if(height <= mult) return b < height ? b : -1;
  const int per_pass = (height + mult - 1) / mult;
  const int row = (b % per_pass) * mult + b / per_pass;
  return row < height ? row : -1;
}

#ifdef ANSEL_HIP_MEASURING
__device__ __forceinline__ float4 vertical5(const float4 *__restrict__ in, const int width, const int height,
                                            const int row, const int col, const int mult, float4 *centre)
{
  const float4 a = in[(size_t)clampi(row - 2 * mult, 0, height - 1) * width + col];
  const float4 b = in[(size_t)clampi(row - mult, 0, height - 1) * width + col];
  const float4 c = in[(size_t)row * width + col];
  const float4 d = in[(size_t)clampi(row + mult, 0, height - 1) * width + col];
  const float4 e = in[(size_t)clampi(row + 2 * mult, 0, height - 1) * width + col];
  if(centre) *centre = c;
  return tap5(a, b, c, d, e);
}

template <int R, int T>
__global__ __launch_bounds__(256) void bspline_decompose(const float4 *__restrict__ in, float4 *__restrict__ hf,
                                                         float4 *__restrict__ lf, const int width, const int height,
                                                         const int mult, const int groups, const int gx)
{
  __shared__ float4 vert[(T + 4) * R + 2];
  const int bx = xcd_col();
  if(bx >= gx) return;
  const int row = walk_row(blockIdx.y, height, mult);
  if(row < 0) return;
  const int group = bx % groups, tile = bx / groups;
  const int r0 = group * R, k0 = tile * T;
  const int tid = threadIdx.x;
  const int r = tid % R, k = tid / R;
  const int col = r0 + r + (k0 + k) * mult;
  float4 centre = make_float4(0.f, 0.f, 0.f, 0.f);
  if(col < width) vert[(k + 2) * R + r] = vertical5(in, width, height, row, col, mult, &centre);
  if(tid < 4 * R)
  {
    const int hr = tid % R, hs = tid / R;
    const int hk = hs < 2 ? hs - 2 : T + hs - 2;
    const int hcol = r0 + hr + (k0 + hk) * mult;
    if(hcol >= 0 && hcol < width) vert[(hk + 2) * R + hr] = vertical5(in, width, height, row, hcol, mult, nullptr);
  }
  else if(tid == 4 * R)
    vert[(T + 4) * R] = vertical5(in, width, height, row, 0, mult, nullptr);
  else if(tid == 4 * R + 1)
    vert[(T + 4) * R + 1] = vertical5(in, width, height, row, width - 1, mult, nullptr);
  __syncthreads();
  if(col >= width) return;
  float4 t[5];
#pragma unroll
  for(int s = -2; s <= 2; s++)
  {
    const int c = col + s * mult;
    t[s + 2] = c < 0 ? vert[(T + 4) * R] : (c > width - 1 ? vert[(T + 4) * R + 1] : vert[(k + s + 2) * R + r]);
  }
  const float4 low = tap5(t[0], t[1], t[2], t[3], t[4]);
  const size_t o = (size_t)row * width + col;
  lf[o] = low;
  nt_store(hf + o, make_float4(centre.x - low.x, centre.y - low.y, centre.z - low.z, centre.w - low.w));
}
#endif

template <int R, int T>
__global__ __launch_bounds__(256) void bspline_decompose_strip(const float4 *__restrict__ in, float4 *__restrict__ hf,
                                                               float4 *__restrict__ lf, const int width, const int height,
                                                               const int mult, const int groups, const int strip,
                                                               const int strips_per_class, const unsigned *__restrict__ gate)
{
  if(gate && *gate == 0u) return;
  __shared__ float4 vert[2][(T + 4) * R + 2];
  const int bx = blockIdx.x;
  const int cls = blockIdx.y / strips_per_class, k0s = (blockIdx.y - cls * strips_per_class) * strip;
  const int n_cls = (height - cls + mult - 1) / mult;
  if(k0s >= n_cls) return;
  const int nrows = (strip < n_cls - k0s) ? strip : n_cls - k0s;
  const int r_first = cls + k0s * mult;
  const int group = bx % groups, tile = bx / groups;
  const int r0 = group * R, k0 = tile * T;
  const int tid = threadIdx.x;
  const int r = tid % R, k = tid / R;
  const int col = r0 + r + (k0 + k) * mult;
  const bool own = col < width;
  int col2 = -1, slot2 = 0;
  if(tid < 4 * R)
  {
    const int hr = tid % R, hs = tid / R;
    const int hk = hs < 2 ? hs - 2 : T + hs - 2;
    const int hcol = r0 + hr + (k0 + hk) * mult;
    if(hcol >= 0 && hcol < width)
    {
      col2 = hcol;
      slot2 = (hk + 2) * R + hr;
    }
  }
  else if(tid == 4 * R)
  {
    col2 = 0;
    slot2 = (T + 4) * R;
  }
  else if(tid == 4 * R + 1)
  {
    col2 = width - 1;
    slot2 = (T + 4) * R + 1;
  }
  const bool second = col2 >= 0;
#define BS_ROW(q) ((size_t)clampi(r_first + (q) * mult, 0, height - 1) * width)
  const float4 z = make_float4(0.f, 0.f, 0.f, 0.f);
  float4 a = z, b = z, c = z, d = z, e = z, a2 = z, b2 = z, c2 = z, d2 = z, e2 = z;
  if(own)
  {
    a = in[BS_ROW(-2) + col];
    b = in[BS_ROW(-1) + col];
    c = in[BS_ROW(0) + col];
    d = in[BS_ROW(1) + col];
    e = in[BS_ROW(2) + col];
  }
  if(second)
  {
    a2 = in[BS_ROW(-2) + col2];
    b2 = in[BS_ROW(-1) + col2];
    c2 = in[BS_ROW(0) + col2];
    d2 = in[BS_ROW(1) + col2];
    e2 = in[BS_ROW(2) + col2];
  }
  for(int kk = 0; kk < nrows; kk++)
  {
    const int row = r_first + kk * mult;
    const bool more = kk + 1 < nrows;
    float4 n1 = z, n2 = z;
    if(more && own) n1 = in[BS_ROW(kk + 3) + col];
    if(more && second) n2 = in[BS_ROW(kk + 3) + col2];
    float4 *const V = vert[kk & 1];
    if(own) V[(k + 2) * R + r] = tap5(a, b, c, d, e);
    if(second) V[slot2] = tap5(a2, b2, c2, d2, e2);
    __syncthreads();
    if(own)
    {
      float4 t[5];
#pragma unroll
      for(int s = -2; s <= 2; s++)
      {
        const int cc = col + s * mult;
        t[s + 2] = cc < 0 ? V[(T + 4) * R] : (cc > width - 1 ? V[(T + 4) * R + 1] : V[(k + s + 2) * R + r]);
      }
      const float4 low = tap5(t[0], t[1], t[2], t[3], t[4]);
      const size_t o = (size_t)row * width + col;
      lf[o] = low;
      if(hf) nt_store(hf + o, make_float4(c.x - low.x, c.y - low.y, c.z - low.z, c.w - low.w));
    }
    a = b;
    b = c;
    c = d;
    d = e;
    e = n1;
    a2 = b2;
    b2 = c2;
    c2 = d2;
    d2 = e2;
    e2 = n2;
  }
#undef BS_ROW
}

struct bs_px3
{
  float x, y, z;
};
__device__ __forceinline__ bs_px3 tap5(const bs_px3 a, const bs_px3 b, const bs_px3 c, const bs_px3 d, const bs_px3 e)
{
  return { tap5(a.x, b.x, c.x, d.x, e.x), tap5(a.y, b.y, c.y, d.y, e.y), tap5(a.z, b.z, c.z, d.z, e.z) };
}
template <int R, int T, bool IN4>
__global__ __launch_bounds__(256) void bspline_decompose_strip3(const void *__restrict__ in_v, bs_px3 *__restrict__ lf,
                                                                const int width, const int height, const int strip,
                                                                const int strips_per_class, unsigned *__restrict__ alpha_flag)
{
  static_assert(R * T == 256, "a workgroup's columns: one span of 256");
  constexpr int mult = R;
  if(!IN4 && *alpha_flag != 0u) return;
  __shared__ bs_px3 vert[2][(T + 4) * R + 2];
  const float4 *const in4 = static_cast<const float4 *>(in_v);
  const bs_px3 *const in3 = static_cast<const bs_px3 *>(in_v);
  unsigned alpha_bits = 0;
  auto at = [&](const size_t i) -> bs_px3 {
    if constexpr(IN4)
    {
      const float4 v = in4[i];
      alpha_bits |= __float_as_uint(v.w);
      return { v.x, v.y, v.z };
    }
    else
      return in3[i];
  };
  const int cls = blockIdx.y / strips_per_class, k0s = (blockIdx.y - cls * strips_per_class) * strip;
  const int n_cls = (height - cls + mult - 1) / mult;
  if(k0s >= n_cls) return;
  const int nrows = (strip < n_cls - k0s) ? strip : n_cls - k0s;
  const int r_first = cls + k0s * mult;
  const int k0 = (int)blockIdx.x * T;
  const int tid = threadIdx.x;
  const int r = tid % R, k = tid / R;
  const int col = r + (k0 + k) * mult;
  const bool own = col < width;
  int col2 = -1, slot2 = 0;
  if(tid < 4 * R)
  {
    const int hr = tid % R, hs = tid / R;
    const int hk = hs < 2 ? hs - 2 : T + hs - 2;
    const int hcol = hr + (k0 + hk) * mult;
    if(hcol >= 0 && hcol < width)
    {
      col2 = hcol;
      slot2 = (hk + 2) * R + hr;
    }
  }
  else if(tid == 4 * R)
  {
    col2 = 0;
    slot2 = (T + 4) * R;
  }
  else if(tid == 4 * R + 1)
  {
    col2 = width - 1;
    slot2 = (T + 4) * R + 1;
  }
  const bool second = col2 >= 0;
#define BS_ROW(q) ((size_t)clampi(r_first + (q) * mult, 0, height - 1) * width)
  const bs_px3 z = { 0.f, 0.f, 0.f };
  bs_px3 a = z, b = z, c = z, d = z, e = z, a2 = z, b2 = z, c2 = z, d2 = z, e2 = z;
  if(own)
  {
    a = at(BS_ROW(-2) + col);
    b = at(BS_ROW(-1) + col);
    c = at(BS_ROW(0) + col);
    d = at(BS_ROW(1) + col);
    e = at(BS_ROW(2) + col);
  }
  if(second)
  {
    a2 = at(BS_ROW(-2) + col2);
    b2 = at(BS_ROW(-1) + col2);
    c2 = at(BS_ROW(0) + col2);
    d2 = at(BS_ROW(1) + col2);
    e2 = at(BS_ROW(2) + col2);
  }
  for(int kk = 0; kk < nrows; kk++)
  {
    const int row = r_first + kk * mult;
    const bool more = kk + 1 < nrows;
    bs_px3 n1 = z, n2 = z;
    if(more && own) n1 = at(BS_ROW(kk + 3) + col);
    if(more && second) n2 = at(BS_ROW(kk + 3) + col2);
    bs_px3 *const V = vert[kk & 1];
    if(own) V[(k + 2) * R + r] = tap5(a, b, c, d, e);
    if(second) V[slot2] = tap5(a2, b2, c2, d2, e2);
    __syncthreads();
    if(own)
    {
      bs_px3 t[5];
#pragma unroll
      for(int s = -2; s <= 2; s++)
      {
        const int cc = col + s * mult;
        t[s + 2] = cc < 0 ? V[(T + 4) * R] : (cc > width - 1 ? V[(T + 4) * R + 1] : V[(k + s + 2) * R + r]);
      }
      lf[(size_t)row * width + col] = tap5(t[0], t[1], t[2], t[3], t[4]);
    }
    a = b;
    b = c;
    c = d;
    d = e;
    e = n1;
    a2 = b2;
    b2 = c2;
    c2 = d2;
    d2 = e2;
    e2 = n2;
  }
#undef BS_ROW
  if(IN4 && __builtin_amdgcn_ballot_w64(alpha_bits != 0u) != 0ull && (tid & 63) == 0) atomicOr(alpha_flag, 1u);
}

#ifdef ANSEL_HIP_MEASURING
__device__ __forceinline__ float4 bs_row_taps(const float4 *__restrict__ V, const int col, const int step, const int origin,
                                              const int width)
{
  float4 t[5];
#pragma unroll
  for(int j = 0; j < 5; j++) t[j] = V[clampi(col + (j - 2) * step, 0, width - 1) - origin];
  return tap5(t[0], t[1], t[2], t[3], t[4]);
}

template <int M, int AHEAD>
__global__ __launch_bounds__(320) void bspline_decompose2_strip(const float4 *__restrict__ in, float4 *__restrict__ low1,
                                                                float4 *__restrict__ low2, const int width, const int height,
                                                                const int strip, const int strips_per_class)
{
  constexpr int M2 = 2 * M, WA = 256 + 12 * M, WB = 256 + 8 * M;
  static_assert(WA <= 320, "a lane a column");
  __shared__ float4 VA[2][WA], VC[2][WB];
  const int c0 = (int)blockIdx.x * 256;
  const int cls = blockIdx.y / strips_per_class, k0s = (blockIdx.y - cls * strips_per_class) * strip;
  const int n_cls = (height - cls + M2 - 1) / M2;
  if(k0s >= n_cls) return;
  const int nrows = (strip < n_cls - k0s) ? strip : n_cls - k0s;
  const int r_first = cls + k0s * M2;
  const int tid = threadIdx.x;
  const int ca = c0 - 6 * M + tid, cb = c0 - 4 * M + tid;
  const bool on_a = tid < WA && ca >= 0 && ca < width;
  const bool on_b = tid < WB && cb >= 0 && cb < width;
  const bool on_c = on_b && tid >= 4 * M && tid < 4 * M + 256;
  const float4 z = make_float4(0.f, 0.f, 0.f, 0.f);
  float4 a = z, b = z, c = z, d = z, e = z;
  float4 nd[AHEAD], ne[AHEAD];
  float4 r0 = z, r1 = z, r2 = z, r3 = z, r4 = z;
  bool rolling = false;
#define BS_AT(r) in[(size_t)clampi((r), 0, height - 1) * width + ca]
  const int ca_safe = clampi(ca, 0, width - 1);
#define BS_SAFE(r) in[(size_t)clampi((r), 0, height - 1) * width + ca_safe]
#pragma unroll
  for(int j = 0; j < AHEAD; j++)
  {
    const int sj = r_first + (j - 2) * M2;
    nd[j] = BS_SAFE(sj + M);
    ne[j] = BS_SAFE(sj + 2 * M);
  }
#define BS_STEP(kk, J) \
  { \
    const int k = (kk); \
    const int q = k + 5, sig = r_first + (q - 2) * M2, buf = q & 1; \
    const bool produce = q <= nrows + 3; \
    if(produce) \
    { \
      if(sig >= 0 && sig < height) \
      { \
        if(rolling) \
        { \
          a = c; \
          b = d; \
          c = e; \
        } \
        else \
        { \
          if(on_a) \
          { \
            a = BS_AT(sig - 2 * M); \
            b = BS_AT(sig - M); \
            c = BS_AT(sig); \
          } \
          rolling = true; \
        } \
        d = nd[J]; \
        e = ne[J]; \
        if(on_a) VA[buf][tid] = tap5(a, b, c, d, e); \
      } \
      else \
      { \
         \
        rolling = false; \
        const int tau = clampi(sig, 0, height - 1); \
        if(on_a) VA[buf][tid] = tap5(BS_AT(tau - 2 * M), BS_AT(tau - M), BS_AT(tau), BS_AT(tau + M), BS_AT(tau + 2 * M)); \
      } \
    } \
     \
    nd[J] = BS_SAFE(sig + AHEAD * M2 + M); \
    ne[J] = BS_SAFE(sig + AHEAD * M2 + 2 * M); \
    if(k >= 0 && on_b) VC[buf][tid] = tap5(r0, r1, r2, r3, r4); \
    __syncthreads(); \
    if(k >= 0 && on_c) low2[(size_t)(r_first + k * M2) * width + cb] = bs_row_taps(VC[buf], cb, M2, c0 - 4 * M, width); \
    if(produce) \
    { \
      r0 = r1; \
      r1 = r2; \
      r2 = r3; \
      r3 = r4; \
      if(on_b) \
      { \
        r4 = bs_row_taps(VA[buf], cb, M, c0 - 6 * M, width); \
        if(on_c && q >= 2 && q - 2 < nrows) low1[(size_t)sig * width + cb] = r4; \
      } \
    } \
  }
  for(int k0 = -5; k0 < nrows; k0 += AHEAD)
  {
    BS_STEP(k0, 0)
    if constexpr(AHEAD > 1)
      if(k0 + 1 < nrows) BS_STEP(k0 + 1, 1)
    if constexpr(AHEAD > 2)
      if(k0 + 2 < nrows) BS_STEP(k0 + 2, 2)
    if constexpr(AHEAD > 3)
      if(k0 + 3 < nrows) BS_STEP(k0 + 3, 3)
  }
#undef BS_STEP
#undef BS_AT
#undef BS_SAFE
}
#endif

}

namespace ansel
{
#ifdef ANSEL_HIP_MEASURING
int bspline_launch_decompose2(int devid, hipStream_t s, const float4 *in, float4 *low1, float4 *low2, int w, int h, int mult)
{
  (void)devid;
  if(mult != 1 && mult != 4) return DT_HIP_INVALID_ARG;
  const int m2 = 2 * mult;
  const int classes = h < m2 ? h : m2, per_class = (h + m2 - 1) / m2;
  const int gx = (w + 255) / 256;
  const int strip = strip_rows(gx, classes, per_class, 64);
  const int spc = (per_class + strip - 1) / strip;
  const dim3 grid(gx, classes * spc);
  launch_scope ls(devid, "diffuse_decompose");
  static const char *const ahead_env = measuring_env("ANSEL_HIP_BSPLINE_AHEAD");
  const int ahead = ahead_env ? atoi(ahead_env) : 1;
#define BS_PAIR(MM) \
  switch(ahead) \
  { \
    case 2: bspline_decompose2_strip<MM, 2><<<grid, 320, 0, s>>>(in, low1, low2, w, h, strip, spc); break; \
    case 4: bspline_decompose2_strip<MM, 4><<<grid, 320, 0, s>>>(in, low1, low2, w, h, strip, spc); break; \
    case 3: bspline_decompose2_strip<MM, 3><<<grid, 320, 0, s>>>(in, low1, low2, w, h, strip, spc); break; \
    default: bspline_decompose2_strip<MM, 1><<<grid, 320, 0, s>>>(in, low1, low2, w, h, strip, spc); break; \
  }
  if(mult == 1)
  {
    BS_PAIR(1);
  }
  else
  {
    BS_PAIR(4);
  }
#undef BS_PAIR
  return check_launch("diffuse_decompose");
}
#endif

int bspline_launch_decompose3(int devid, hipStream_t s, const void *in, bool in4, float *lf, int w, int h, int mult, unsigned *alpha_flag)
{
  (void)devid;
  if(mult != 1 && mult != 2 && mult != 4 && mult != 8 && mult != 16) return DT_HIP_INVALID_ARG;
  if(in4 && mult != 1) return DT_HIP_INVALID_ARG;
  const int classes = h < mult ? h : mult, per_class = (h + mult - 1) / mult;
  const int gx = (w + 255) / 256;
  const int strip = strip_rows(gx, classes, per_class);
  const int spc = (per_class + strip - 1) / strip;
  const dim3 grid(gx, classes * spc);
  launch_scope ls(devid, "diffuse_decompose");
  bs_px3 *const out = reinterpret_cast<bs_px3 *>(lf);
  if(in4) bspline_decompose_strip3<1, 256, true><<<grid, 256, 0, s>>>(in, out, w, h, strip, spc, alpha_flag);
  else if(mult == 1) bspline_decompose_strip3<1, 256, false><<<grid, 256, 0, s>>>(in, out, w, h, strip, spc, alpha_flag);
  else if(mult == 2) bspline_decompose_strip3<2, 128, false><<<grid, 256, 0, s>>>(in, out, w, h, strip, spc, alpha_flag);
  else if(mult == 4) bspline_decompose_strip3<4, 64, false><<<grid, 256, 0, s>>>(in, out, w, h, strip, spc, alpha_flag);
  else if(mult == 8) bspline_decompose_strip3<8, 32, false><<<grid, 256, 0, s>>>(in, out, w, h, strip, spc, alpha_flag);
  else bspline_decompose_strip3<16, 16, false><<<grid, 256, 0, s>>>(in, out, w, h, strip, spc, alpha_flag);
  return check_launch("diffuse_decompose");
}

int bspline_launch_decompose(int devid, hipStream_t s, const float4 *in, float4 *hf, float4 *lf, int w, int h, int mult,
                             const unsigned *gate)
{
  const int steps = (w + mult - 1) / mult;
  launch_scope ls(devid, "diffuse_decompose");
#ifdef ANSEL_HIP_MEASURING
  static const bool per_row = getenv("ANSEL_HIP_BSPLINE_PER_ROW") != nullptr;
  if(per_row)
  {
    const int rows = (h <= mult) ? h : ((h + mult - 1) / mult) * mult;
    if(mult == 1)
      bspline_decompose<1, 256><<<dim3(xcd_pad((steps + 255) / 256), rows), 256, 0, s>>>(in, hf, lf, w, h, mult, 1, (steps + 255) / 256);
    else if(mult == 2)
      bspline_decompose<2, 128><<<dim3(xcd_pad((steps + 127) / 128), rows), 256, 0, s>>>(in, hf, lf, w, h, mult, 1, (steps + 127) / 128);
    else if(mult == 4)
      bspline_decompose<4, 64><<<dim3(xcd_pad((steps + 63) / 64), rows), 256, 0, s>>>(in, hf, lf, w, h, mult, 1, (steps + 63) / 64);
    else
    {
      const int groups = mult / 8;
      bspline_decompose<8, 32><<<dim3(xcd_pad(((steps + 31) / 32) * groups), rows), 256, 0, s>>>(in, hf, lf, w, h, mult, groups,
                                                                                            ((steps + 31) / 32) * groups);
    }
    return check_launch("diffuse_decompose");
  }
#endif
  const int classes = h < mult ? h : mult, per_class = (h + mult - 1) / mult;
  const int gx = mult == 1 ? (steps + 255) / 256 : (mult == 2 ? (steps + 127) / 128 : (mult == 4 ? (steps + 63) / 64 : ((steps + 31) / 32) * (mult / 8)));
  const int strip = strip_rows(gx, classes, per_class);
  const int spc = (per_class + strip - 1) / strip;
  const dim3 grid(gx, classes * spc);
  if(mult == 1) bspline_decompose_strip<1, 256><<<grid, 256, 0, s>>>(in, hf, lf, w, h, mult, 1, strip, spc, gate);
  else if(mult == 2) bspline_decompose_strip<2, 128><<<grid, 256, 0, s>>>(in, hf, lf, w, h, mult, 1, strip, spc, gate);
  else if(mult == 4) bspline_decompose_strip<4, 64><<<grid, 256, 0, s>>>(in, hf, lf, w, h, mult, 1, strip, spc, gate);
  else bspline_decompose_strip<8, 32><<<grid, 256, 0, s>>>(in, hf, lf, w, h, mult, mult / 8, strip, spc, gate);
  return check_launch("diffuse_decompose");
}
}
```

### ansel_amd/csrc/hip_common.h

```cpp
#pragma once
#include <hip/hip_runtime.h>
#include <stdint.h>
#include <stdio.h>
#include <string.h>
#include "ansel_hip.h"
#include "dev_buf.h"

#ifdef ANSEL_HIP_MEASURING
#include <stdlib.h>
static inline const char *measuring_env(const char *name) { return getenv(name); }
#else
static inline constexpr const char *measuring_env(const char *) { return nullptr; }
#endif

namespace ansel
{

enum dispatch_key_t
{
  DISPATCH_NLM_V2 = 0,
  DISPATCH_NLM_FUSED,
  DISPATCH_AMAZE_UNFUSED,
  DISPATCH_AMAZE_SLAB,
  DISPATCH_AMAZE_BLOCKS,
  DISPATCH_BILAT_BLUR_SPLIT,
  DISPATCH_STRIP_ROWS,
  DISPATCH_KEYS
};
int dispatch_override(dispatch_key_t key);

static inline int strip_rows(const int gx, const int classes, const int per_class, const int longest = 32)
{
  const int forced = dispatch_override(DISPATCH_STRIP_ROWS);
  if(forced) return forced;
  int strip = longest;
  while(strip > 4 && (size_t)gx * classes * ((per_class + strip - 1) / strip) < 2048) strip /= 2;
  return strip;
}

void set_last_error(const char *fmt, ...);

hipStream_t stream_of(int devid);
int upload_small(int devid, void *dst_dev, const void *src_host, size_t bytes);
bool make_current(int devid);
int hip_device_of(int devid);
bool valid_device(int devid);

struct launch_scope
{
  int devid;
  const char *tag;
  hipEvent_t start, stop;
  bool active;
  launch_scope(int devid, const char *tag);
  ~launch_scope();
};

static inline int check_launch(const char *what)
{
  const hipError_t e = hipGetLastError();
  if(e != hipSuccess)
  {
    set_last_error("%s: %s", what, hipGetErrorString(e));
    return DT_HIP_DEFAULT_ERROR;
  }
  return DT_HIP_SUCCESS;
}

#define ANSEL_HIP_CHECK(expr)                                                                   \
  do                                                                                            \
  {                                                                                             \
    const hipError_t _e = (expr);                                                               \
    if(_e != hipSuccess)                                                                        \
    {                                                                                           \
      ansel::set_last_error("%s:%d %s: %s", __FILE__, __LINE__, #expr, hipGetErrorString(_e));  \
      return DT_HIP_DEFAULT_ERROR;                                                              \
    }                                                                                           \
  } while(0)

typedef float v4f_t __attribute__((ext_vector_type(4)));
__device__ __forceinline__ void nt_store(float4 *p, const float4 v)
{
  const v4f_t t = { v.x, v.y, v.z, v.w };
  __builtin_nontemporal_store(t, reinterpret_cast<v4f_t *>(p));
}

template <typename T> __device__ __forceinline__ const T &kernarg_at(const int offset)
{
  typedef const T __attribute__((address_space(4))) *p4;
  return *(const T *)(p4)((const char __attribute__((address_space(4))) *)__builtin_amdgcn_kernarg_segment_ptr() + offset);
}
template <typename T, typename... Before> constexpr int kernarg_offset_after()
{
  size_t off = 0;
  ((off = (off + alignof(Before) - 1) / alignof(Before) * alignof(Before) + sizeof(Before)), ...);
  return (int)((off + alignof(T) - 1) / alignof(T) * alignof(T));
}

static inline unsigned xcd_pad(const int gx) { return (unsigned)((gx + 7) / 8) * 8; }
__device__ __forceinline__ int xcd_col() { return (int)((blockIdx.x + blockIdx.y / 64) % gridDim.x); }

#define HL_MIN_CLIPPED 25
struct hl_journal
{
  unsigned long long count;
  unsigned long long index[HL_MIN_CLIPPED];
  float value[HL_MIN_CLIPPED];
};
int highlights_resolve_launch(int devid, float *out, const hl_journal *journal);

struct rcd_band_t
{
  int tv0, tv1;
  int in_row0, in_rows;
  int out_row0, out_rows;
};

struct band_view_t
{
  int frame_h;
  int buf_row0;
  int row0, row1;
};
int nlmeans_halo_rows(const dt_hip_piece_t *piece, const dt_hip_nlmeans_data_t *d);
int nlmeans_process_band(int devid, const dt_hip_piece_t *piece, const dt_hip_nlmeans_data_t *d, const band_view_t *band,
                         dt_hip_mem_t dev_in, dt_hip_mem_t dev_out);
int diffuse_halo_rows(const dt_hip_piece_t *piece, const dt_hip_diffuse_data_t *d);
int diffuse_process_rows(int devid, const dt_hip_piece_t *piece, const dt_hip_diffuse_data_t *d, int first_row,
                         dt_hip_mem_t dev_in, dt_hip_mem_t dev_out);
int diffuse_process_post_lab(int devid, const dt_hip_piece_t *piece, const dt_hip_diffuse_data_t *d, dt_hip_mem_t dev_in,
                             dt_hip_mem_t dev_out, const dt_hip_lab_data_t *lab);
int denoiseprofile_halo_rows(const dt_hip_piece_t *piece, const dt_hip_denoiseprofile_data_t *d);
struct dn_band_job_t;
int denoiseprofile_band_begin(int devid, const dt_hip_piece_t *piece, const dt_hip_denoiseprofile_data_t *d,
                              const band_view_t *band, int buf_rows, dt_hip_mem_t dev_in, dt_hip_mem_t dev_out,
                              dn_band_job_t **job);
int denoiseprofile_band_step(dn_band_job_t *job, dt_hip_mem_t *halo_buf, int *halo_rows, double **sums, size_t *sum_count);
int denoiseprofile_band_finish(dn_band_job_t *job, dt_hip_mem_t dev_out);
void denoiseprofile_band_abort(dn_band_job_t *job);
int guided_filter_launch(int devid, const float4 *guide, float *mask, int width, int height, int w, float sqrt_eps,
                         float guide_weight, float minv, float maxv);
int detail_refine_launch(int devid, const float *rawdetail, const float *form, float fill, float level, int width, int height,
                         float *refined);
int bilat_band_supported(const dt_hip_piece_t *piece, const dt_hip_bilat_data_t *d);
int blend_refines_with_detail_mask(const dt_hip_blend_data_t *d);
int bilat_band_begin(int devid, const dt_hip_piece_t *piece, const dt_hip_bilat_data_t *d, dt_hip_mem_t *grid, size_t *bytes);
int bilat_band_splat(int devid, const dt_hip_piece_t *piece, const dt_hip_bilat_data_t *d, dt_hip_mem_t grid,
                     dt_hip_mem_t in_rows, int row0, int rows);
int bilat_band_finish(int devid, const dt_hip_piece_t *piece, const dt_hip_bilat_data_t *d, dt_hip_mem_t grid,
                      dt_hip_mem_t in_rows, dt_hip_mem_t out_rows, int row0, int rows);

int file_host_view(const char *who, int devid, void *host, size_t host_bytes, void **view);
int file_to_host_launch(hipStream_t s, const void *dev_file, size_t capacity, void *view, size_t host_bytes);

static inline unsigned stream_grid(size_t work_items, unsigned block)
{
  size_t g = (work_items + block - 1) / block;
  if(g > 2048u * 4u) g = 2048u * 4u;
  if(g < 1) g = 1;
  return (unsigned)g;
}

static inline unsigned pixel_grid(size_t pixels)
{
  const size_t g = (pixels + 255) / 256;
  return (unsigned)(g < 1 ? 1 : (g > 0x7fffffffu ? 0x7fffffffu : g));
}

}
```

### ansel_amd/csrc/runtime.cpp

```cpp
#include "hip_common.h"

#include <algorithm>
#include <atomic>
#include <mutex>
#include <unordered_map>
#include <map>
#include <vector>
#include <string>
#include <stdarg.h>

namespace
{

struct event_rec
{
  const char *tag;
  hipEvent_t start, stop;
};

struct device_t
{
  int hip_id = -1;
  std::string name;
  hipStream_t stream = nullptr;
  bool own_stream = false;
  std::mutex lock;
  bool events_enabled = false;
  std::mutex ev_lock;
  std::vector<event_rec> events;
  std::vector<hipEvent_t> event_pool;
  size_t cur_bytes = 0, peak_bytes = 0;
  std::multimap<size_t, void *> free_pool;
  std::atomic<uint64_t> test_fill{ 0 };
  struct staging_t
  {
    void *host = nullptr;
    size_t cap = 0;
    hipEvent_t ev = nullptr;
    bool used = false;
  };
  std::mutex staging_lock;
  staging_t staging[8];
  int staging_next = 0;
};

struct alloc_t
{
  size_t size;
  int devid;
  int width, height, bpp;
  void *host;
};

std::mutex g_mutex;
bool g_inited = false;
std::vector<device_t *> g_devs;
std::unordered_map<void *, alloc_t> g_allocs;
thread_local char t_error[512] = "";

}

namespace ansel
{

void set_last_error(const char *fmt, ...)
{
  va_list ap;
  va_start(ap, fmt);
  vsnprintf(t_error, sizeof(t_error), fmt, ap);
  va_end(ap);
}

bool valid_device(int devid) { return g_inited && devid >= 0 && devid < (int)g_devs.size(); }

bool make_current(int devid)
{
  if(!valid_device(devid)) return false;
  const int want = g_devs[devid]->hip_id;
  int cur = -1;
  if(hipGetDevice(&cur) == hipSuccess && cur == want) return true;
  return hipSetDevice(want) == hipSuccess;
}

int hip_device_of(int devid) { return valid_device(devid) ? g_devs[devid]->hip_id : -1; }

int upload_small(int devid, void *dst_dev, const void *src_host, size_t bytes)
{
  if(!valid_device(devid) || !dst_dev || (!src_host && bytes)) return DT_HIP_INVALID_ARG;
  if(bytes == 0) return DT_HIP_SUCCESS;
  device_t *d = g_devs[devid];
  if(!make_current(devid)) return DT_HIP_DEFAULT_ERROR;
  std::lock_guard<std::mutex> g(d->staging_lock);
  device_t::staging_t &st = d->staging[d->staging_next];
  d->staging_next = (d->staging_next + 1) % 8;
  if(st.used && hipEventSynchronize(st.ev) != hipSuccess) return DT_HIP_DEFAULT_ERROR;
  if(st.cap < bytes)
  {
    if(st.host) (void)hipHostFree(st.host);
    st.host = nullptr;
    st.cap = 0;
    size_t cap = 4096;
    while(cap < bytes) cap *= 2;
    if(hipHostMalloc(&st.host, cap, hipHostMallocDefault) != hipSuccess)
    {
      set_last_error("upload_small: no pinned staging buffer of %zu bytes", cap);
      st.host = nullptr;
      return DT_HIP_SYSMEM_ALLOCATION;
    }
    st.cap = cap;
  }
  if(!st.ev && hipEventCreateWithFlags(&st.ev, hipEventDisableTiming) != hipSuccess) return DT_HIP_DEFAULT_ERROR;
  memcpy(st.host, src_host, bytes);
  if(hipMemcpyAsync(dst_dev, st.host, bytes, hipMemcpyHostToDevice, d->stream) != hipSuccess || hipEventRecord(st.ev, d->stream) != hipSuccess)
  {
    set_last_error("upload_small: the copy of %zu bytes could not be enqueued", bytes);
    return DT_HIP_DEFAULT_ERROR;
  }
  st.used = true;
  return DT_HIP_SUCCESS;
}

hipStream_t stream_of(int devid)
{
  if(!make_current(devid)) return nullptr;
  return g_devs[devid]->stream;
}

launch_scope::launch_scope(int devid_, const char *tag_) : devid(devid_), tag(tag_), active(false)
{
  if(!valid_device(devid)) return;
  device_t *d = g_devs[devid];
  if(!d->events_enabled) return;
  make_current(devid);
  std::lock_guard<std::mutex> g(d->ev_lock);
  auto get = [&]() {
    hipEvent_t e;
    if(!d->event_pool.empty())
    {
      e = d->event_pool.back();
      d->event_pool.pop_back();
    }
    else if(hipEventCreate(&e) != hipSuccess)
      e = nullptr;
    return e;
  };
  start = get();
  stop = get();
  if(!start || !stop || hipEventRecord(start, d->stream) != hipSuccess)
  {
    (void)hipGetLastError();
    if(start) d->event_pool.push_back(start);
    if(stop) d->event_pool.push_back(stop);
    return;
  }
  active = true;
}

launch_scope::~launch_scope()
{
  if(!active) return;
  device_t *d = g_devs[devid];
  std::lock_guard<std::mutex> g(d->ev_lock);
  if(hipEventRecord(stop, d->stream) != hipSuccess)
  {
    (void)hipGetLastError();
    d->event_pool.push_back(start);
    d->event_pool.push_back(stop);
    return;
  }
  d->events.push_back({ tag, start, stop });
}

}

using namespace ansel;

extern "C" {

const char *dt_hip_last_error(void) { return t_error; }

int dt_hip_init(void)
{
  std::lock_guard<std::mutex> g(g_mutex);
  if(g_inited) return DT_HIP_SUCCESS;
  int n = 0;
  if(hipGetDeviceCount(&n) != hipSuccess || n <= 0)
  {
    set_last_error("dt_hip_init: no HIP device visible");
    return DT_HIP_DEFAULT_ERROR;
  }
  for(int i = 0; i < n; i++)
  {
    hipDeviceProp_t prop;
    if(hipGetDeviceProperties(&prop, i) != hipSuccess) continue;
    device_t *d = new device_t;
    d->hip_id = i;
    d->name = prop.name[0] ? prop.name : prop.gcnArchName;
    if(hipSetDevice(i) != hipSuccess || hipStreamCreateWithFlags(&d->stream, hipStreamNonBlocking) != hipSuccess)
    {
      delete d;
      continue;
    }
    d->own_stream = true;
    g_devs.push_back(d);
  }
  if(g_devs.empty())
  {
    set_last_error("dt_hip_init: no usable HIP device");
    return DT_HIP_DEFAULT_ERROR;
  }
  (void)hipSetDevice(g_devs[0]->hip_id);
  g_inited = true;
  return DT_HIP_SUCCESS;
}

void dt_hip_cleanup(void)
{
  std::lock_guard<std::mutex> g(g_mutex);
  if(!g_inited) return;
  for(device_t *d : g_devs)
  {
    (void)hipSetDevice(d->hip_id);
    (void)hipStreamSynchronize(d->stream);
    for(auto &kv : d->free_pool) (void)hipFree(kv.second);
    for(auto &e : d->events)
    {
      (void)hipEventDestroy(e.start);
      (void)hipEventDestroy(e.stop);
    }
    for(auto e : d->event_pool) (void)hipEventDestroy(e);
    for(auto &st : d->staging)
    {
      if(st.ev) (void)hipEventDestroy(st.ev);
      if(st.host) (void)hipHostFree(st.host);
    }
    if(d->own_stream) (void)hipStreamDestroy(d->stream);
    delete d;
  }
  for(auto &kv : g_allocs)
    if(!kv.second.host) (void)hipFree(kv.first);
  g_allocs.clear();
  g_devs.clear();
  g_inited = false;
}

int dt_hip_is_inited(void) { return g_inited ? 1 : 0; }

int dt_hip_get_num_devices(void) { return g_inited ? (int)g_devs.size() : 0; }

const char *dt_hip_get_device_name(int devid) { return valid_device(devid) ? g_devs[devid]->name.c_str() : ""; }

size_t dt_hip_get_device_available(int devid)
{
  if(!valid_device(devid)) return 0;
  size_t fr = 0, tot = 0;
  make_current(devid);
  if(hipMemGetInfo(&fr, &tot) != hipSuccess) return 0;
  std::lock_guard<std::mutex> g(g_mutex);
  for(auto &kv : g_devs[devid]->free_pool) fr += kv.first;
  return fr;
}

size_t dt_hip_get_device_memalloc(int devid)
{
  return dt_hip_get_device_available(devid);
}

int dt_hip_reserve_device_for_pipe(int pipetype)
{
  (void)pipetype;
  if(!g_inited) return -1;
  for(size_t i = 0; i < g_devs.size(); i++)
    if(g_devs[i]->lock.try_lock()) return (int)i;
  return -1;
}

void dt_hip_reserve_device_by_id(int devid)
{
  if(valid_device(devid)) g_devs[devid]->lock.lock();
}

int dt_hip_try_reserve_device_by_id(int devid)
{
  if(!valid_device(devid)) return 1;
  return g_devs[devid]->lock.try_lock() ? 0 : 1;
}

void dt_hip_release_device(int devid)
{
  if(valid_device(devid)) g_devs[devid]->lock.unlock();
}

int dt_hip_get_device_max_image_size(int devid, int *width, int *height)
{
  if(!valid_device(devid)) return 0;
  if(width) *width = 1 << 20;
  if(height) *height = 1 << 20;
  return 1;
}

size_t dt_hip_get_device_max_global_mem(int devid)
{
  if(!valid_device(devid)) return 0;
  size_t free_b = 0, total_b = 0;
  make_current(devid);
  if(hipMemGetInfo(&free_b, &total_b) != hipSuccess) return 0;
  return total_b;
}

static int g_error_count = 0;
static bool g_stopped = false;
int dt_hip_report_pipe_error(void)
{
  if(!g_inited) return 2;
  std::lock_guard<std::mutex> g(g_mutex);
  g_error_count++;
  if(g_error_count < 5) return 1;
  g_stopped = true;
  return 2;
}

int dt_hip_is_enabled(void) { return (g_inited && !g_stopped) ? 1 : 0; }
int dt_hip_update_settings(void) { return dt_hip_is_enabled(); }

void dt_hip_check_tuning(int devid) { (void)devid; }
int dt_hip_avoid_atomics(int devid) { (void)devid; return 0; }
int dt_hip_micro_nap(int devid) { (void)devid; return 0; }
int dt_hip_use_pinned_memory(int devid) { return valid_device(devid) ? 1 : 0; }
int dt_hip_dev_roundup_width(int size, int devid) { (void)devid; return size; }
int dt_hip_dev_roundup_height(int size, int devid) { (void)devid; return size; }

int dt_hip_image_fits_device(int devid, size_t width, size_t height, unsigned bpp, float factor, size_t overhead)
{
  if(!valid_device(devid)) return 0;
  const double need = (double)width * (double)height * (double)bpp * (double)factor + (double)overhead;
  return need <= (double)dt_hip_get_device_available(devid) ? 1 : 0;
}

int dt_hip_image_fits_device_reason(int devid, size_t width, size_t height, unsigned bpp, float factor, size_t overhead,
                                    size_t *needed, size_t *limit)
{
  if(!valid_device(devid)) return 2;
  const double single = (double)width * (double)height * (double)bpp;
  const double total = single * (double)factor + (double)overhead;
  const size_t avail = dt_hip_get_device_available(devid), memalloc = dt_hip_get_device_memalloc(devid);
  if(single > (double)memalloc)
  {
    if(needed) *needed = (size_t)single;
    if(limit) *limit = memalloc;
    return 1;
  }
  if(needed) *needed = (size_t)total;
  if(limit) *limit = avail;
  return total <= (double)avail ? 0 : 2;
}

void *dt_hip_get_stream(int devid) { return (void *)stream_of(devid); }

int dt_hip_set_stream(int devid, void *stream)
{
  if(!valid_device(devid)) return DT_HIP_INVALID_ARG;
  device_t *d = g_devs[devid];
  make_current(devid);
  if((hipStream_t)stream == d->stream) return DT_HIP_SUCCESS;
  if(d->stream || d->own_stream) (void)hipStreamSynchronize(d->stream);
  if(d->own_stream && d->stream) (void)hipStreamDestroy(d->stream);
  d->stream = (hipStream_t)stream;
  d->own_stream = false;
  return DT_HIP_SUCCESS;
}

dt_hip_mem_t dt_hip_alloc_device_buffer(int devid, size_t size)
{
  if(!valid_device(devid) || size == 0) return nullptr;
  device_t *d = g_devs[devid];
  const size_t rounded = (size + 255) & ~(size_t)255;
  std::unique_lock<std::mutex> g(g_mutex);
  void *p = nullptr;
  auto it = d->free_pool.find(rounded);
  if(it != d->free_pool.end())
  {
    p = it->second;
    d->free_pool.erase(it);
  }
  else
  {
    make_current(devid);
    hipError_t e = hipMalloc(&p, rounded);
    if(e != hipSuccess)
    {
      for(auto &kv : d->free_pool) (void)hipFree(kv.second);
      d->free_pool.clear();
      (void)hipGetLastError();
      e = hipMalloc(&p, rounded);
    }
    if(e != hipSuccess)
    {
      set_last_error("dt_hip_alloc_device_buffer: %zu bytes: %s", rounded, hipGetErrorString(e));
      (void)hipGetLastError();
      return nullptr;
    }
  }
  g_allocs[p] = { rounded, devid, 0, 0, 0, nullptr };
  d->cur_bytes += rounded;
  if(d->cur_bytes > d->peak_bytes) d->peak_bytes = d->cur_bytes;
  g.unlock();
  const uint64_t fill = d->test_fill.load(std::memory_order_relaxed);
  if(fill >> 32)
  {
    make_current(devid);
    if(hipMemsetD32Async((hipDeviceptr_t)p, (int)(uint32_t)fill, rounded / 4, d->stream) != hipSuccess
       || hipStreamSynchronize(d->stream) != hipSuccess)
    {
      set_last_error("dt_hip_alloc_device_buffer: the test fill of %zu bytes failed", rounded);
      (void)hipGetLastError();
      dt_hip_release_mem_object(p);
      return nullptr;
    }
  }
  return p;
}

int dt_hip_test_pool_fill(int devid, int enable, uint32_t pattern)
{
  if(!valid_device(devid)) return -1;
  const uint64_t next = enable ? (((uint64_t)1 << 32) | pattern) : 0;
  return (int)(g_devs[devid]->test_fill.exchange(next, std::memory_order_relaxed) >> 32);
}

dt_hip_mem_t dt_hip_alloc_device(int devid, int width, int height, int bpp)
{
  if(width <= 0 || height <= 0 || bpp <= 0) return nullptr;
  dt_hip_mem_t p = dt_hip_alloc_device_buffer(devid, (size_t)width * (size_t)height * (size_t)bpp);
  if(p)
  {
    std::lock_guard<std::mutex> g(g_mutex);
    alloc_t &a = g_allocs[p];
    a.width = width;
    a.height = height;
    a.bpp = bpp;
  }
  return p;
}

void dt_hip_release_mem_object(dt_hip_mem_t mem)
{
  if(!mem) return;
  std::lock_guard<std::mutex> g(g_mutex);
  auto it = g_allocs.find(mem);
  if(it == g_allocs.end()) return;
  const alloc_t a = it->second;
  g_allocs.erase(it);
  if(a.host) return;
  if(a.devid >= 0 && a.devid < (int)g_devs.size())
  {
    device_t *d = g_devs[a.devid];
    d->cur_bytes -= a.size;
    d->free_pool.insert({ a.size, mem });
  }
  else
    (void)hipFree(mem);
}

size_t dt_hip_get_mem_object_size(dt_hip_mem_t mem)
{
  std::lock_guard<std::mutex> g(g_mutex);
  auto it = g_allocs.find(mem);
  return it == g_allocs.end() ? 0 : it->second.size;
}

static alloc_t alloc_of(dt_hip_mem_t mem)
{
  std::lock_guard<std::mutex> g(g_mutex);
  auto it = g_allocs.find(mem);
  return it == g_allocs.end() ? alloc_t{ 0, -1, 0, 0, 0, nullptr } : it->second;
}
int dt_hip_get_image_width(dt_hip_mem_t mem) { return alloc_of(mem).width; }
int dt_hip_get_image_height(dt_hip_mem_t mem) { return alloc_of(mem).height; }
int dt_hip_get_image_element_size(dt_hip_mem_t mem) { return alloc_of(mem).bpp; }
int dt_hip_get_mem_context_id(dt_hip_mem_t mem) { return alloc_of(mem).devid; }

dt_hip_mem_t dt_hip_alloc_device_use_host_pointer(int devid, int width, int height, int bpp, void *host, int flags)
{
  (void)flags;
  if(!valid_device(devid) || !host || width <= 0 || height <= 0 || bpp <= 0 || !dt_hip_is_pinned_memory(host)) return nullptr;
  void *dev = nullptr;
  make_current(devid);
  if(hipHostGetDevicePointer(&dev, host, 0) != hipSuccess || !dev)
  {
    (void)hipGetLastError();
    return nullptr;
  }
  std::lock_guard<std::mutex> g(g_mutex);
  g_allocs[dev] = { (size_t)width * height * bpp, devid, width, height, bpp, host };
  return dev;
}

void *dt_hip_map_buffer(int devid, dt_hip_mem_t buffer, int blocking, int flags, size_t offset, size_t size)
{
  (void)flags;
  (void)size;
  const alloc_t a = alloc_of(buffer);
  if(!a.host || !valid_device(devid)) return nullptr;
  if(blocking && hipStreamSynchronize(stream_of(devid)) != hipSuccess) return nullptr;
  return (char *)a.host + offset;
}
void *dt_hip_map_image(int devid, dt_hip_mem_t buffer, int blocking, int flags, size_t width, size_t height, int bpp)
{
  (void)width;
  (void)height;
  (void)bpp;
  return dt_hip_map_buffer(devid, buffer, blocking, flags, 0, 0);
}
int dt_hip_unmap_mem_object(int devid, dt_hip_mem_t mem, void *mapped_ptr)
{
  (void)mapped_ptr;
  return (valid_device(devid) && alloc_of(mem).host) ? DT_HIP_SUCCESS : DT_HIP_INVALID_ARG;
}

dt_hip_mem_t dt_hip_copy_host_to_device_rowpitch(int devid, void *host, int width, int height, int bpp, int rowpitch)
{
  dt_hip_mem_t d = dt_hip_alloc_device(devid, width, height, bpp);
  if(!d) return nullptr;
  if(dt_hip_write_host_to_device_rowpitch(devid, host, d, width, height, bpp, (size_t)rowpitch, 1) != DT_HIP_SUCCESS)
  {
    dt_hip_release_mem_object(d);
    return nullptr;
  }
  return d;
}
dt_hip_mem_t dt_hip_copy_host_to_device(int devid, void *host, int width, int height, int bpp)
{
  return dt_hip_copy_host_to_device_rowpitch(devid, host, width, height, bpp, 0);
}
dt_hip_mem_t dt_hip_copy_host_to_device_constant(int devid, size_t size, void *host)
{
  dt_hip_mem_t d = dt_hip_alloc_device_buffer(devid, size);
  if(!d) return nullptr;
  if(dt_hip_write_buffer_to_device(devid, host, d, 0, size, 1) != DT_HIP_SUCCESS)
  {
    dt_hip_release_mem_object(d);
    return nullptr;
  }
  return d;
}
int dt_hip_copy_device_to_host(int devid, void *host, dt_hip_mem_t device, int width, int height, int bpp)
{
  return dt_hip_read_host_from_device(devid, host, device, width, height, bpp);
}

int dt_hip_read_buffer_from_device(int devid, void *host, dt_hip_mem_t device, size_t offset, size_t size, int blocking)
{
  if(!valid_device(devid) || !host || !device) return DT_HIP_INVALID_ARG;
  if(!size) return DT_HIP_SUCCESS;
  hipStream_t s = stream_of(devid);
  ANSEL_HIP_CHECK(hipMemcpyAsync(host, (const char *)device + offset, size, hipMemcpyDeviceToHost, s));
  if(blocking) ANSEL_HIP_CHECK(hipStreamSynchronize(s));
  return DT_HIP_SUCCESS;
}
int dt_hip_write_buffer_to_device(int devid, const void *host, dt_hip_mem_t device, size_t offset, size_t size, int blocking)
{
  if(!valid_device(devid) || !host || !device) return DT_HIP_INVALID_ARG;
  if(!size) return DT_HIP_SUCCESS;
  hipStream_t s = stream_of(devid);
  ANSEL_HIP_CHECK(hipMemcpyAsync((char *)device + offset, host, size, hipMemcpyHostToDevice, s));
  if(blocking || dt_hip_is_pinned_memory(host)) ANSEL_HIP_CHECK(hipStreamSynchronize(s));
  return DT_HIP_SUCCESS;
}

int dt_hip_enqueue_barrier(int devid) { return valid_device(devid) ? DT_HIP_SUCCESS : DT_HIP_INVALID_ARG; }

void dt_hip_memory_statistics(int devid, size_t *current, size_t *peak)
{
// ... 306 lines not shown
```

### ansel_amd/csrc/testhooks.hip

```cpp
#include "hip_common.h"
#include "devmath.h"
#include "ieee_inrange.h"

#include <atomic>
#include <string.h>

using namespace ansel;

namespace
{
std::atomic<int> g_dispatch[DISPATCH_KEYS];
const char *const g_dispatch_names[DISPATCH_KEYS] = { "nlm_v2", "nlm_fused", "amaze_unfused", "amaze_slab", "amaze_blocks",
                                                       "bilat_blur_split", "strip_rows" };
}
namespace ansel
{
int dispatch_override(const dispatch_key_t key) { return g_dispatch[key].load(std::memory_order_relaxed); }
}
extern "C" int dt_hip_test_dispatch(const char *key, int value)
{
  if(!key) return DT_HIP_INVALID_ARG;
  for(int k = 0; k < DISPATCH_KEYS; k++)
    if(!strcmp(key, g_dispatch_names[k]))
    {
      if(k == DISPATCH_STRIP_ROWS && value != 0 && value != 4 && value != 8 && value != 16 && value != 32) return DT_HIP_INVALID_ARG;
      g_dispatch[k].store(value);
      return DT_HIP_SUCCESS;
    }
  return DT_HIP_INVALID_ARG;
}

extern "C" int dt_hip_test_strip_rows(int gx, int classes, int per_class) { return strip_rows(gx, classes, per_class); }

namespace
{
template <int FN>
__global__ void devmath_test(const float *__restrict__ x, const float *__restrict__ y, float *__restrict__ o, const size_t n)
{
  for(size_t k = (size_t)blockIdx.x * blockDim.x + threadIdx.x; k < n; k += (size_t)gridDim.x * blockDim.x)
  {
    float r;
    if(FN == 0) r = ansel_math::powf_exact(x[k], y[k]);
    else if(FN == 1) r = ansel_math::log2f_exact(x[k]);
    else if(FN == 2) r = ansel_math::exp2f_exact(x[k]);
    else if(FN == 3) r = ansel_math::expf_exact(x[k]);
    else if(FN == 4) r = ansel_math::atan2f_exact(x[k], y[k]);
    else if(FN == 5) r = ansel_math::hypotf_exact(x[k], y[k]);
    else if(FN == 6) r = ansel_math::sinf_exact(x[k]);
    else if(FN == 7) r = ansel_math::cosf_exact(x[k]);
    else if(FN == 9) r = ansel_math::logf_exact(x[k]);
    else if(FN == 10) r = ansel_ieee::div_core(x[k], y[k]);
    else if(FN == 11) r = ansel_ieee::rcp_core(x[k]);
    else if(FN == 12) r = ansel_ieee::sqrt_core(x[k]);
    else if(FN == 13) r = ansel_ieee::zero_or_above_2m96(x[k]) ? 1.0f : 0.0f;
    else if(FN == 14) r = ansel_ieee::div_uniform(x[k], y[k], ansel_ieee::rcp_refined(y[k]));
    else r = fmodf(x[k], y[k]);
    o[k] = r;
  }
}
template <int FN> int devmath_launch(int devid, const void *x, const void *y, void *o, size_t n)
{
  if(!valid_device(devid)) return DT_HIP_INVALID_ARG;
  devmath_test<FN><<<stream_grid(n, 256), 256, 0, stream_of(devid)>>>((const float *)x, (const float *)y, (float *)o, n);
  return check_launch("devmath_test");
}
}
extern "C" {
int dt_hip_test_powf(int devid, const void *x, const void *y, void *o, size_t n) { return devmath_launch<0>(devid, x, y, o, n); }
int dt_hip_test_log2f(int devid, const void *x, const void *y, void *o, size_t n) { return devmath_launch<1>(devid, x, y, o, n); }
int dt_hip_test_exp2f(int devid, const void *x, const void *y, void *o, size_t n) { return devmath_launch<2>(devid, x, y, o, n); }
int dt_hip_test_expf(int devid, const void *x, const void *y, void *o, size_t n) { return devmath_launch<3>(devid, x, y, o, n); }
int dt_hip_test_atan2f(int devid, const void *x, const void *y, void *o, size_t n) { return devmath_launch<4>(devid, x, y, o, n); }
int dt_hip_test_hypotf(int devid, const void *x, const void *y, void *o, size_t n) { return devmath_launch<5>(devid, x, y, o, n); }
int dt_hip_test_sinf(int devid, const void *x, const void *y, void *o, size_t n) { return devmath_launch<6>(devid, x, y, o, n); }
int dt_hip_test_cosf(int devid, const void *x, const void *y, void *o, size_t n) { return devmath_launch<7>(devid, x, y, o, n); }
int dt_hip_test_fmodf(int devid, const void *x, const void *y, void *o, size_t n) { return devmath_launch<8>(devid, x, y, o, n); }
int dt_hip_test_logf(int devid, const void *x, const void *y, void *o, size_t n) { return devmath_launch<9>(devid, x, y, o, n); }
int dt_hip_test_div_core(int devid, const void *x, const void *y, void *o, size_t n) { return devmath_launch<10>(devid, x, y, o, n); }
int dt_hip_test_rcp_core(int devid, const void *x, const void *y, void *o, size_t n) { return devmath_launch<11>(devid, x, y, o, n); }
int dt_hip_test_sqrt_core(int devid, const void *x, const void *y, void *o, size_t n) { return devmath_launch<12>(devid, x, y, o, n); }
int dt_hip_test_zero_or_above_2m96(int devid, const void *x, const void *y, void *o, size_t n) { return devmath_launch<13>(devid, x, y, o, n); }
int dt_hip_test_div_uniform(int devid, const void *x, const void *y, void *o, size_t n) { return devmath_launch<14>(devid, x, y, o, n); }
}

namespace
{
__global__ __launch_bounds__(64) void lds_dma_x3_test(const float *__restrict__ src, unsigned *__restrict__ dst, const unsigned base)
{
  __shared__ unsigned lds[512];
  for(int i = threadIdx.x; i < 512; i += 64) lds[i] = 0xdeadbeefu;
  __syncthreads();
  using lds_u32_ptr = __attribute__((address_space(3))) unsigned *;
  const unsigned m0v = (unsigned)__builtin_amdgcn_readfirstlane((int)(unsigned)(__UINTPTR_TYPE__)(lds_u32_ptr)lds) + base;
  const unsigned voff = (63u - threadIdx.x) * 12u;
  unsigned keep;
  asm volatile("s_waitcnt lgkmcnt(0)\n\ts_nop 4\n\ts_mov_b32 %0, m0\n\t"
               "s_mov_b32 m0, %3\n\ts_nop 0\n\tglobal_load_lds_dwordx3 %1, %2\n\t"
               "s_mov_b32 m0, %0\n\ts_waitcnt vmcnt(0)"
               : "=&s"(keep)
               : "v"(voff), "s"(src), "s"(m0v)
               : "memory");
  __syncthreads();
  for(int i = threadIdx.x; i < 512; i += 64) dst[i] = lds[i];
}
}
extern "C" int dt_hip_test_lds_dma_x3(int devid, const void *src, void *dst, unsigned base)
{
  if(!valid_device(devid) || !src || !dst || base % 4 != 0 || base + 1024 > 2048) return DT_HIP_INVALID_ARG;
  lds_dma_x3_test<<<1, 64, 0, stream_of(devid)>>>((const float *)src, (unsigned *)dst, base);
  return check_launch("lds_dma_x3_test");
}
```

### ansel_amd/lib.py

```python
import ctypes as C
import os

from . import abi

HERE = os.path.dirname(os.path.abspath(__file__))
LIB_PATH = os.environ.get("ANSEL_HIP_LIB") or os.path.join(HERE, "libansel_hip.so")

_lib = None
_env_fill = False
_env_fill_applied = False


class AnselHipError(RuntimeError):
    pass


def load():
    global _lib
    if _lib is not None:
        return _lib
    if not os.path.exists(LIB_PATH):
        if os.environ.get("ANSEL_HIP_LIB"):
            raise AnselHipError(
                "ANSEL_HIP_LIB=%s does not exist: the measuring build is made by `python -m ansel_amd.build --measuring` "
# ... 6 lines not shown
            import torch
        except Exception:
            pass
    lib = C.CDLL(LIB_PATH)
    vp, i, u, sz = C.c_void_p, C.c_int, C.c_uint32, C.c_size_t
    P = C.POINTER
    protos = {
        "dt_hip_init": (i, []),
        "dt_hip_cleanup": (None, []),
        "dt_hip_is_inited": (i, []),
        "dt_hip_get_num_devices": (i, []),
        "dt_hip_get_device_name": (C.c_char_p, [i]),
        "dt_hip_get_device_available": (sz, [i]),
        "dt_hip_get_device_memalloc": (sz, [i]),
        "dt_hip_reserve_device_for_pipe": (i, [i]),
        "dt_hip_reserve_device_by_id": (None, [i]),
        "dt_hip_try_reserve_device_by_id": (i, [i]),
        "dt_hip_release_device": (None, [i]),
        "dt_hip_get_device_max_image_size": (i, [i, P(i), P(i)]),
        "dt_hip_get_device_max_global_mem": (sz, [i]),
        "dt_hip_report_pipe_error": (i, []),
        "dt_hip_is_enabled": (i, []),
        "dt_hip_update_settings": (i, []),
        "dt_hip_check_tuning": (None, [i]),
        "dt_hip_avoid_atomics": (i, [i]),
        "dt_hip_micro_nap": (i, [i]),
        "dt_hip_use_pinned_memory": (i, [i]),
        "dt_hip_dev_roundup_width": (i, [i, i]),
        "dt_hip_dev_roundup_height": (i, [i, i]),
        "dt_hip_image_fits_device_reason": (i, [i, sz, sz, C.c_uint, C.c_float, sz, P(sz), P(sz)]),
        "dt_hip_get_image_width": (i, [vp]),
        "dt_hip_get_image_height": (i, [vp]),
        "dt_hip_get_image_element_size": (i, [vp]),
        "dt_hip_get_mem_context_id": (i, [vp]),
        "dt_hip_alloc_device_use_host_pointer": (vp, [i, i, i, i, vp, i]),
        "dt_hip_map_buffer": (vp, [i, vp, i, i, sz, sz]),
        "dt_hip_map_image": (vp, [i, vp, i, i, sz, sz, i]),
        "dt_hip_unmap_mem_object": (i, [i, vp, vp]),
        "dt_hip_copy_host_to_device": (vp, [i, vp, i, i, i]),
        "dt_hip_copy_host_to_device_rowpitch": (vp, [i, vp, i, i, i, i]),
        "dt_hip_copy_host_to_device_constant": (vp, [i, sz, vp]),
        "dt_hip_copy_device_to_host": (i, [i, vp, vp, i, i, i]),
        "dt_hip_read_buffer_from_device": (i, [i, vp, vp, sz, sz, i]),
        "dt_hip_write_buffer_to_device": (i, [i, vp, vp, sz, sz, i]),
        "dt_hip_enqueue_barrier": (i, [i]),
        "dt_hip_events_wait_for": (None, [i]),
        "dt_hip_events_flush": (i, [i, i]),
        "dt_hip_image_fits_device": (i, [i, sz, sz, C.c_uint, C.c_float, sz]),
        "dt_hip_get_stream": (vp, [i]),
        "dt_hip_set_stream": (i, [i, vp]),
        "dt_hip_alloc_device": (vp, [i, i, i, i]),
        "dt_hip_alloc_device_buffer": (vp, [i, sz]),
        "dt_hip_release_mem_object": (None, [vp]),
        "dt_hip_get_mem_object_size": (sz, [vp]),
        "dt_hip_memory_statistics": (None, [i, P(sz), P(sz)]),
        "dt_hip_write_host_to_device": (i, [i, vp, vp, i, i, i]),
        "dt_hip_write_host_to_device_rowpitch": (i, [i, vp, vp, i, i, i, sz, i]),
        "dt_hip_read_host_from_device": (i, [i, vp, vp, i, i, i]),
        "dt_hip_read_host_from_device_rowpitch": (i, [i, vp, vp, i, i, i, sz, i]),
        "dt_hip_enqueue_copy_buffer_to_buffer": (i, [i, vp, vp, sz, sz, sz]),
        "dt_hip_read_host_from_device_raw": (i, [i, vp, vp, P(sz), P(sz), i, i]),
        "dt_hip_write_host_to_device_raw": (i, [i, vp, vp, P(sz), P(sz), i, i]),
        "dt_hip_enqueue_copy_image": (i, [i, vp, vp, P(sz), P(sz), P(sz)]),
        "dt_hip_enqueue_copy_region": (i, [i, vp, i, i, i, vp, i, i, i, i, i, i]),
        "dt_hip_finish": (i, [i]),
        "dt_hip_events_enable": (None, [i, i]),
        "dt_hip_events_reset": (None, [i]),
        "dt_hip_events_profiling": (i, [i, P(C.c_char_p), P(C.c_float), P(i), i]),
        "dt_hip_last_error": (C.c_char_p, []),
        "dt_hip_abi_sizeof": (sz, [C.c_char_p]),
        "dt_hip_crop_dcraw_filters": (u, [u, u, u]),
        "dt_hip_iop_rawprepare_process": (i, [i, P(abi.Piece), P(abi.RawprepareData), vp, vp]),
        "dt_hip_iop_temperature_process": (i, [i, P(abi.Piece), P(abi.TemperatureData), vp, vp]),
        "dt_hip_iop_highlights_process": (i, [i, P(abi.Piece), P(abi.HighlightsData), vp, vp]),
        "dt_hip_iop_demosaic_process": (i, [i, P(abi.Piece), P(abi.DemosaicData), vp, vp]),
        "dt_hip_iop_demosaic_tiling": (None, [P(abi.Piece), P(abi.DemosaicData), P(abi.Tiling)]),
        "dt_hip_iop_exposure_process": (i, [i, P(abi.Piece), P(abi.ExposureData), vp, vp]),
        "dt_hip_iop_colorin_process": (i, [i, P(abi.Piece), P(abi.Conversion), vp, vp]),
        "dt_hip_iop_colorout_process": (i, [i, P(abi.Piece), P(abi.Conversion), vp, vp]),
        "dt_hip_iop_channelmixerrgb_process": (i, [i, P(abi.Piece), P(abi.ChannelmixerrgbData), vp, vp]),
        "dt_hip_iop_filmicrgb_process": (i, [i, P(abi.Piece), P(abi.FilmicrgbData), vp, vp]),
        "dt_hip_iop_diffuse_process": (i, [i, P(abi.Piece), P(abi.DiffuseData), vp, vp]),
        "dt_hip_iop_denoiseprofile_process": (i, [i, P(abi.Piece), P(abi.DenoiseprofileData), vp, vp]),
        "dt_hip_iop_nlmeans_process": (i, [i, P(abi.Piece), P(abi.NlmeansData), vp, vp]),
        "dt_hip_iop_detailmask_process": (i, [i, P(abi.Piece), P(abi.DetailmaskData), vp, vp]),
        "dt_hip_transform_rgb_to_lab": (i, [i, P(abi.Piece), P(abi.LabData), vp, vp]),
        "dt_hip_transform_lab_to_rgb": (i, [i, P(abi.Piece), P(abi.LabData), vp, vp]),
        "dt_hip_iop_bilat_process": (i, [i, P(abi.Piece), P(abi.BilatData), vp, vp]),
        "dt_hip_iop_finalscale_process": (i, [i, P(abi.Piece), P(abi.FinalscaleData), vp, vp]),
        "dt_hip_iop_initialscale_process": (i, [i, P(abi.Piece), P(abi.FinalscaleData), vp, vp]),
        "dt_hip_iop_flip_process": (i, [i, P(abi.Piece), P(abi.FlipData), vp, vp]),
        "dt_hip_iop_flip_modify_roi_out": (i, [P(abi.FlipData), i, i, P(abi.Roi), P(abi.Roi)]),
        "dt_hip_iop_flip_modify_roi_in": (i, [P(abi.FlipData), i, i, P(abi.Roi), P(abi.Roi)]),
        "dt_hip_iop_flip_distort_transform": (i, [P(abi.FlipData), i, i, P(C.c_float), sz]),
        "dt_hip_iop_flip_distort_backtransform": (i, [P(abi.FlipData), i, i, P(C.c_float), sz]),
        "dt_hip_raw_unpack": (i, [i, vp, i, i, C.c_size_t, i, i, vp]),
        "dt_hip_develop_blend_process": (i, [i, P(abi.Piece), P(abi.BlendData), vp, vp]),
        "dt_hip_iop_basebuffer_process": (i, [i, P(abi.Piece), i, i, i, vp, vp]),
        "dt_hip_alloc_host_pinned": (vp, [sz]),
        "dt_hip_free_host_pinned": (None, [vp]),
        "dt_hip_is_pinned_memory": (i, [vp]),
        "dt_hip_plan_tiles_ptp": (i, [i, i, i, i, P(abi.Tiling), C.c_uint, sz, sz, i, i, P(abi.TilePlan)]),
        "dt_hip_default_process_tiling_ptp": (i, [i, C.c_char_p, P(abi.Piece), vp, sz, P(abi.Tiling), vp, vp, i, i, sz]),
        "dt_hip_default_tiling": (None, [P(abi.Piece), i, P(abi.Tiling)]),
        "dt_hip_plan_tiles_roi": (i, [P(abi.Roi), P(abi.Roi), i, i, P(abi.Tiling), C.c_uint, sz, sz, i, i, P(abi.TilePlanRoi)]),
        "dt_hip_tile_rois_finalscale": (i, [P(abi.TilePlanRoi), P(abi.Roi), P(abi.Roi), i, i, P(abi.Roi), P(abi.Roi), P(abi.Roi)]),
        "dt_hip_tile_rois_flip": (i, [P(abi.TilePlanRoi), P(abi.Roi), P(abi.Roi), P(abi.FlipData), i, i, P(abi.Roi), P(abi.Roi),
                                      P(abi.Roi)]),
        "dt_hip_default_process_tiling_roi": (i, [i, C.c_char_p, P(abi.Piece), vp, sz, P(abi.Tiling), vp, vp, i, i, sz]),
        "dt_hip_iop_denoiseprofile_tiling": (None, [P(abi.Piece), P(abi.DenoiseprofileData), P(abi.Tiling)]),
        "dt_hip_iop_nlmeans_tiling": (None, [P(abi.Piece), P(abi.NlmeansData), P(abi.Tiling)]),
        "dt_hip_iop_bilat_tiling": (None, [P(abi.Piece), P(abi.BilatData), P(abi.Tiling)]),
        "dt_hip_iop_diffuse_tiling": (None, [P(abi.Piece), P(abi.DiffuseData), P(abi.Tiling)]),
        "dt_hip_export_convert_u16": (i, [i, i, i, vp, vp]),
        "dt_hip_export_convert_u8": (i, [i, i, i, vp, vp]),
        "dt_hip_export_pack_rows": (i, [i, i, i, i, i, vp, vp]),
        "dt_hip_jpeg_bound": (sz, [i, i, P(abi.JpegData)]),
        "dt_hip_export_jpeg": (i, [i, i, i, P(abi.JpegData), vp, vp]),
        "dt_hip_png_bound": (sz, [i, i, P(abi.PngData)]),
        "dt_hip_export_png": (i, [i, i, i, P(abi.PngData), vp, vp]),
        "dt_hip_tiff_bound": (sz, [i, i, P(abi.TiffData)]),
        "dt_hip_export_tiff": (i, [i, i, i, P(abi.TiffData), vp, vp]),
        "dt_hip_webp_bound": (sz, [i, i, P(abi.WebpData)]),
        "dt_hip_export_webp": (i, [i, i, i, P(abi.WebpData), vp, vp]),
        "dt_hip_pipe_new": (vp, [i]),
        "dt_hip_pipe_free": (None, [vp]),
        "dt_hip_pipe_add_node": (i, [vp, C.c_char_p, P(abi.Piece), vp, sz]),
        "dt_hip_pipe_set_fusion": (None, [vp, i]),
        "dt_hip_pipe_num_groups": (i, [vp]),
        "dt_hip_pipe_process": (i, [vp, vp, vp]),
        "dt_hip_batch_new": (vp, [vp, i, sz, sz]),
        "dt_hip_batch_free": (None, [vp]),
        "dt_hip_batch_submit": (i, [vp, vp, vp]),
        "dt_hip_batch_wait": (i, [vp, i]),
        "dt_hip_batch_drain": (i, [vp]),
        "dt_hip_batch_set_writer": (i, [vp, vp, vp]),
        "dt_hip_batch_set_file_output": (i, [vp, sz]),
        "dt_hip_batch_file_bytes": (i, [vp, i, P(sz)]),
        "dt_hip_read_file_to_host": (i, [i, vp, sz, vp, sz]),
        "dt_hip_plan_bands": (i, [i, i, i, i, P(abi.Band)]),
        "dt_hip_band_halo_rows": (i, [C.c_char_p, P(abi.Piece), vp, sz]),
        "dt_hip_pipe_band_begin": (i, [vp, P(abi.Band), vp, P(abi.BandState)]),
        "dt_hip_pipe_band_resolve": (i, [vp, P(abi.Band), P(abi.BandState)]),
        "dt_hip_pipe_band_finish": (i, [vp, P(abi.Band), P(abi.BandState), vp]),
        "dt_hip_pipe_band_relay": (i, [vp, P(abi.Band), P(abi.BandState)]),
        "dt_hip_pipe_band_abort": (None, [vp, P(abi.BandState)]),
        "dt_hip_pipe_process_bands": (i, [P(vp), i, P(abi.Band), P(vp), P(vp)]),
        "dt_hip_pipe_bands_stats": (None, [P(abi.BandStats)]),
        "dt_hip_peer_selftest": (i, [P(i), i]),
        "dt_hip_iop_highlights_process_deferred": (i, [i, P(abi.Piece), P(abi.HighlightsData), vp, vp, vp]),
        "dt_hip_iop_highlights_resolve": (i, [i, vp, vp]),
        "dt_hip_test_dispatch": (i, [C.c_char_p, i]),
        "dt_hip_test_strip_rows": (i, [i, i, i]),
        "dt_hip_test_nlm_last": (i, [P(i)]),
        "dt_hip_test_pool_fill": (i, [i, i, u]),
    }
    missing = []
    for name, (res, args) in protos.items():
        try:
            fn = getattr(lib, name)
        except AttributeError:
            missing.append(name)
            continue
        fn.restype = res
        fn.argtypes = args
    lib._ansel_missing = missing
    lib._ansel_protos = protos
    _lib = lib
    return lib


def test_dispatch(key, value):
    check(load().dt_hip_test_dispatch(key.encode(), int(value)), "dt_hip_test_dispatch(%s)" % key)


def test_strip_rows(gx, classes, per_class):
    return load().dt_hip_test_strip_rows(int(gx), int(classes), int(per_class))


def test_pool_fill(devid, enable, pattern=0):
    was = load().dt_hip_test_pool_fill(devid, 1 if enable else 0, int(pattern) & 0xFFFFFFFF)
    if was < 0:
        raise AnselHipError("dt_hip_test_pool_fill: no device %d" % devid)
    return bool(was)


NLM_BODIES = ("none", "tall", "v4", "v3", "v2", "pipelined", "staged", "global")


def test_nlm_last():
    out = (C.c_int * 8)()
    check(load().dt_hip_test_nlm_last(out), "dt_hip_test_nlm_last")
    keys = ("body", "tight", "deep", "radius", "npatch", "reach", "n_border", "nchunks")
    d = dict(zip(keys, list(out)))
    d["body"] = NLM_BODIES[d["body"]]
    return d


def check(rc, what=""):
    if rc != abi.DT_HIP_SUCCESS:
        msg = load().dt_hip_last_error()
        raise AnselHipError("%s failed with %d: %s" % (what, rc, msg.decode() if msg else ""))


def init():
    lib = load()
    if lib._ansel_missing:
        raise AnselHipError("libansel_hip.so lacks symbols declared in include/ansel_hip.h: %s"
                            % ", ".join(lib._ansel_missing))
    check(lib.dt_hip_init(), "dt_hip_init")
    global _env_fill_applied
    if not _env_fill_applied:
        _env_fill_applied = True
        if env_pool_fill() is not None:
            test_pool_fill(0, True, env_pool_fill())
    return lib


def env_pool_fill():
    global _env_fill
    if _env_fill is False:
        env = os.environ.get("ANSEL_TEST_POOL_FILL")
        _env_fill = (int(env, 16) & 0xFFFFFFFF) if env else None
    return _env_fill


class DeviceBuffer:

    def __init__(self, devid, nbytes):
        self.lib = load()
        self.devid = devid
        self.nbytes = int(nbytes)
        self.ptr = self.lib.dt_hip_alloc_device_buffer(devid, self.nbytes)
        if not self.ptr:
            raise AnselHipError("device allocation of %d bytes failed: %s"
                                % (self.nbytes, self.lib.dt_hip_last_error().decode()))

    @classmethod
    def from_numpy(cls, devid, arr):
        import numpy as np
        arr = np.ascontiguousarray(arr)
        b = cls(devid, arr.nbytes)
        check(b.lib.dt_hip_write_buffer_to_device(devid, arr.ctypes.data_as(C.c_void_p), b.ptr, 0, arr.nbytes, 1),
              "write_buffer_to_device")
        return b

    def upload(self, arr):
        import numpy as np
        arr = np.ascontiguousarray(arr)
        assert arr.nbytes <= self.nbytes
        check(self.lib.dt_hip_write_buffer_to_device(self.devid, arr.ctypes.data_as(C.c_void_p), self.ptr, 0, arr.nbytes, 1),
              "write_buffer_to_device")

    def to_numpy(self, shape, dtype):
        import numpy as np
        out = np.empty(shape, dtype=dtype)
        assert out.nbytes <= self.nbytes
        check(self.lib.dt_hip_read_buffer_from_device(self.devid, out.ctypes.data_as(C.c_void_p), self.ptr, 0,
                                                      out.nbytes, 1), "read_buffer_from_device")
        return out

    def release(self):
        if self.ptr:
            self.lib.dt_hip_release_mem_object(self.ptr)
            self.ptr = None

    def __del__(self):
        try:
            self.release()
        except Exception:
            pass
```

Before: 1617.

## Split tail strips into shorter pieces sized to device residency

Adds a strip plan that keeps most strip-walking blocks at full length and splits the last ones into shorter pieces. How many are split depends on occupancy-derived resident block counts per kernel, queried once and cached. The goal is to shrink the wave-quantization tail where a few long strips run alone on an otherwise idle GPU. The cost is extra halo re-reads and more blocks in the tail, plus some index math per block.

Result: no change. 1628 (median of 6 runs) (+0.7%).

```diff
diff --git a/ansel_amd/csrc/denoiseprofile.hip b/ansel_amd/csrc/denoiseprofile.hip
--- a/ansel_amd/csrc/denoiseprofile.hip
+++ b/ansel_amd/csrc/denoiseprofile.hip
@@ -424,7 +424,8 @@
   double *partial;
   int width, height, mult_arg;
   float inv_sigma2;
-  int nseg, in_row0, in_rows, strip, strips_per_class;
+  int nseg, in_row0, in_rows;
+  strip_plan_t plan;
   vst_args fa;
   unsigned *alpha_flag;
   int flag_sense;
@@ -441,7 +442,7 @@
                                                           float4 *__restrict__ detail, double *__restrict__ partial,
                                                           const int width, const int height, const int mult_arg,
                                                           const float inv_sigma2, const int nseg, const int in_row0,
-                                                          const int in_rows, const int strip, const int strips_per_class,
+                                                          const int in_rows, const strip_plan_t plan,
                                                           const vst_args fa_by_value, unsigned *__restrict__ alpha_flag, const int flag_sense)
 {
   const vst_args &fa = kernarg_at<vst_args>((int)offsetof(dn_strip_kernargs, fa));
@@ -477,10 +478,11 @@
   };
   __shared__ double runs[2][4][4];
   const int bx = blockIdx.x;
-  const int cls = blockIdx.y / strips_per_class, k0 = (blockIdx.y - cls * strips_per_class) * strip;
+  const strip_block_t sb = strip_of_block(plan, blockIdx.y);
+  const int cls = sb.cls, k0 = sb.k0;
   const int n_cls = (height - cls + mult - 1) / mult;
   if(k0 >= n_cls) return;
-  const int nrows = min(strip, n_cls - k0);
+  const int nrows = min(sb.rows, n_cls - k0);
   const int r_first = cls + k0 * mult;
   const int tw = 256 + 4 * mult;
   extern __shared__ float4 ring[];
@@ -623,7 +625,7 @@
   if(ALPHA0 && alpha_flag && __builtin_amdgcn_ballot_w64(alpha_bits != 0) != 0ull && lane == 0) atomicOr(alpha_flag, 1u);
 }
 
-static void launch_decompose(hipStream_t st, const float4 *in, float4 *coarse, float4 *detail, double *partial, const int width,
+static void launch_decompose(const int devid, hipStream_t st, const float4 *in, float4 *coarse, float4 *detail, double *partial, const int width,
                              const int height, const int mult, const float inv_sigma2, const int nseg, const int in_row0,
                              const int in_rows, const vst_args *pre = nullptr, unsigned *alpha_flag = nullptr, const int mode = 0)
 {
@@ -639,8 +641,6 @@
 #endif
   const int classes = height < mult ? height : mult, per_class = (height + mult - 1) / mult;
   const int strip = strip_rows(nseg, classes, per_class);
-  const int strips_per_class = (per_class + strip - 1) / strip;
-  const dim3 grid(nseg, classes * strips_per_class);
   size_t lds = (size_t)DN_RING * (256 + 4 * mult) * sizeof(float);
 #ifdef ANSEL_HIP_MEASURING
   static const char *const pad_env = measuring_env("ANSEL_HIP_DN_LDS_PAD");
@@ -651,15 +651,17 @@
 #define DN_LDS(A0_) (lds * ((A0_) ? 3 : 4) + lds_pad)
   vst_args none;
   memset(&none, 0, sizeof(none));
-#define DN_LAUNCH_(PRE_, M_, A0_, FA_, SENSE_)                                                                                          \
-  dn_decompose_strip<PRE_, M_, A0_><<<grid, 256, DN_LDS(A0_), st>>>(in, coarse, detail, partial, width, height, mult, inv_sigma2, nseg, in_row0, \
-                                                            in_rows, strip, strips_per_class, FA_, alpha_flag, SENSE_)
+  auto launch = [&](auto kernel, const size_t bytes, const vst_args &fa, const int sense) {
+    const strip_plan_t plan = strip_plan(nseg, classes, per_class, strip, strip_resident(devid, (const void *)kernel, bytes));
+    kernel<<<dim3(nseg, strip_plan_blocks(plan, classes)), 256, bytes, st>>>(in, coarse, detail, partial, width, height, mult, inv_sigma2, nseg,
+                                                                             in_row0, in_rows, plan, fa, alpha_flag, sense);
+  };
+#define DN_LAUNCH_(PRE_, M_, A0_, FA_, SENSE_) launch(dn_decompose_strip<PRE_, M_, A0_>, DN_LDS(A0_), FA_, SENSE_)
 #define DN_LAUNCH(PRE_, M_, FA_)                  \
   do                                              \
   {                                               \
     if(mode == 1)                                 \
-      dn_decompose_strip<PRE_, M_, true, true><<<grid, 256, DN_LDS(true), st>>>(in, coarse, detail, partial, width, height, mult, inv_sigma2, nseg, in_row0, \
-                                                            in_rows, strip, strips_per_class, FA_, alpha_flag, 0); \
+      launch(dn_decompose_strip<PRE_, M_, true, true>, DN_LDS(true), FA_, 0); \
     else if(mode == 2)                            \
       DN_LAUNCH_(PRE_, M_, false, FA_, 2);        \
     else if(alpha_flag && (PRE_))                 \
@@ -1182,7 +1184,7 @@
   const float sigma_band = powf(varf, scale) * 1.0f;
   {
     launch_scope ls(devid, "dn_decompose");
-    launch_decompose(st, j->cur.as<float4>(), coarse.as<float4>() + (size_t)top * w, j->det[scale].as<float4>(), j->local.as<double>(), w, j->rows, mult,
+    launch_decompose(devid, st, j->cur.as<float4>(), coarse.as<float4>() + (size_t)top * w, j->det[scale].as<float4>(), j->local.as<double>(), w, j->rows, mult,
                      1.0f / (sigma_band * sigma_band), nseg, j->cur_top, j->cur_top + j->rows + j->cur_bottom);
   }
   int err = check_launch("denoiseprofile band decompose");
@@ -1329,7 +1331,7 @@
       const float sigma_band = powf(varf, scale) * 1.0f;
       {
         launch_scope ls(devid, "dn_decompose");
-        launch_decompose(st, b1, coarse[scale], scale == 0 ? det0 : nullptr, partial + (size_t)scale * n_partial * 4, w, h, mult,
+        launch_decompose(devid, st, b1, coarse[scale], scale == 0 ? det0 : nullptr, partial + (size_t)scale * n_partial * 4, w, h, mult,
                          1.0f / (sigma_band * sigma_band), nseg, 0, h, scale == 0 ? &fa : nullptr, alpha_flag, alpha_flag ? seq + 1 : 0);
       }
       err = check_launch("denoiseprofile band");
diff --git a/ansel_amd/csrc/diffuse.hip b/ansel_amd/csrc/diffuse.hip
--- a/ansel_amd/csrc/diffuse.hip
+++ b/ansel_amd/csrc/diffuse.hip
@@ -426,18 +426,19 @@
 template <bool HSUB, int MODE, bool DMA, int L3>
 __device__ __forceinline__ void pde_strip_body(const float4 *__restrict__ hf, const float4 *__restrict__ hsub,
                                                const float4 *__restrict__ lf, float4 *__restrict__ out, const pde_args &a,
-                                               const int final_pass, const unsigned char *__restrict__ mask, const int strip,
-                                               const int strips_per_class)
+                                               const int final_pass, const unsigned char *__restrict__ mask,
+                                               const strip_plan_t &plan)
 {
   static_assert(L3 == 0 || (HSUB && DMA), "three-float planes: the low-pass chain's LDS-DMA form only");
   if(a.gate && ((*a.gate != 0u) == (a.gate_sense == 1))) return;
   extern __shared__ float4 r2s[];
   pde_px3 *const r2s3 = reinterpret_cast<pde_px3 *>(r2s);
   const int mult = a.mult;
-  const int cls = blockIdx.y / strips_per_class, k0s = (blockIdx.y - cls * strips_per_class) * strip;
+  const strip_block_t sb = strip_of_block(plan, blockIdx.y);
+  const int cls = sb.cls, k0s = sb.k0;
   const int n_cls = (a.height - cls + mult - 1) / mult;
   if(k0s >= n_cls) return;
-  const int nrows = (strip < n_cls - k0s) ? strip : n_cls - k0s;
+  const int nrows = (sb.rows < n_cls - k0s) ? sb.rows : n_cls - k0s;
   const int r_first = cls + k0s * mult;
   const int tx = threadIdx.x, tw = 256 + 2 * mult;
   const int col = (int)blockIdx.x * 256 + tx;
@@ -676,17 +677,16 @@
 __global__ __launch_bounds__(256, 3) void diffuse_pde_strip(const float4 *__restrict__ hf, const float4 *__restrict__ hsub,
                                                          const float4 *__restrict__ lf,
                                                          float4 *__restrict__ out, const pde_args a, const int final_pass,
-                                                         const unsigned char *__restrict__ mask, const int strip,
-                                                         const int strips_per_class)
-{
-  pde_strip_body<HSUB, MODE, DMA, 0>(hf, hsub, lf, out, a, final_pass, mask, strip, strips_per_class);
+                                                         const unsigned char *__restrict__ mask, const strip_plan_t plan)
+{
+  pde_strip_body<HSUB, MODE, DMA, 0>(hf, hsub, lf, out, a, final_pass, mask, plan);
 }
 template <int MODE, bool H0_4>
 __global__ __launch_bounds__(256, 3) void diffuse_pde_strip3(const float4 *__restrict__ hf, const float4 *__restrict__ hsub,
                                                           const float4 *__restrict__ lf, float4 *__restrict__ out, const pde_args a,
-                                                          const int final_pass, const int strip, const int strips_per_class)
-{
-  pde_strip_body<true, MODE, true, H0_4 ? 2 : 1>(hf, hsub, lf, out, a, final_pass, nullptr, strip, strips_per_class);
+                                                          const int final_pass, const strip_plan_t plan)
+{
+  pde_strip_body<true, MODE, true, H0_4 ? 2 : 1>(hf, hsub, lf, out, a, final_pass, nullptr, plan);
 }
 
 __device__ __forceinline__ uint32_t splitmix32(const uint64_t seed)
@@ -901,8 +901,8 @@
   }
 }
 
-typedef void (*pde_strip_fn)(const float4 *, const float4 *, const float4 *, float4 *, pde_args, int, const unsigned char *, int, int);
-typedef void (*pde_strip3_fn)(const float4 *, const float4 *, const float4 *, float4 *, pde_args, int, int, int);
+typedef void (*pde_strip_fn)(const float4 *, const float4 *, const float4 *, float4 *, pde_args, int, const unsigned char *, strip_plan_t);
+typedef void (*pde_strip3_fn)(const float4 *, const float4 *, const float4 *, float4 *, pde_args, int, strip_plan_t);
 
 template <int MD> static pde_strip_fn pde_strip_forms(const bool chain, const bool dma)
 {
@@ -940,7 +940,6 @@
   if(strip_env) longest = atoi(strip_env);
 #endif
   const int strip = strip_rows(gx, classes, per_class, longest);
-  const int spc = (per_class + strip - 1) / strip;
   size_t ring = (size_t)PDE_RING * (256 + 2 * a.mult) * sizeof(float4);
 #ifdef ANSEL_HIP_MEASURING
   static const char *const pad_env = measuring_env("ANSEL_HIP_PDE_LDS_PAD");
@@ -948,15 +947,21 @@
 #endif
   static const bool generic = measuring_env("ANSEL_HIP_PDE_GENERIC") != nullptr;
   const int mode = generic ? -1 : pde_mode_of(a);
-  const dim3 sgrid(gx, classes * spc);
+  auto plan_of = [&](const void *const kernel, const size_t bytes) {
+    return strip_plan(gx, classes, per_class, strip, strip_resident(j.devid, kernel, bytes));
+  };
   if(p3)
   {
     const size_t lds3 = (size_t)PDE_RING * (256 + 2 * a.mult) * 12 + (size_t)4 * 3 * (64 + 2 * a.mult) * 16;
-    pde_strip3_kernel(mode, h0_4)<<<sgrid, 256, lds3, j.st>>>(h0, h1, cur, to, a, final_pass, strip, spc);
+    const pde_strip3_fn kernel = pde_strip3_kernel(mode, h0_4);
+    const strip_plan_t plan = plan_of((const void *)kernel, lds3);
+    kernel<<<dim3(gx, strip_plan_blocks(plan, classes)), 256, lds3, j.st>>>(h0, h1, cur, to, a, final_pass, plan);
     return;
   }
   const size_t lds = dma ? ring + (size_t)4 * 3 * (64 + 2 * a.mult) * sizeof(float4) : ring;
-  pde_strip_kernel(mode, chain, dma)<<<sgrid, 256, lds, j.st>>>(h0, h1, cur, to, a, final_pass, j.p.mask.as<unsigned char>(), strip, spc);
+  const pde_strip_fn kernel = pde_strip_kernel(mode, chain, dma);
+  const strip_plan_t plan = plan_of((const void *)kernel, lds);
+  kernel<<<dim3(gx, strip_plan_blocks(plan, classes)), 256, lds, j.st>>>(h0, h1, cur, to, a, final_pass, j.p.mask.as<unsigned char>(), plan);
 }
 
 static int diffuse_iteration(const diffuse_job_t &j, pde_args &a, const bool p3, const bool first, const bool last,
diff --git a/ansel_amd/csrc/diffuse_bspline.hip b/ansel_amd/csrc/diffuse_bspline.hip
--- a/ansel_amd/csrc/diffuse_bspline.hip
+++ b/ansel_amd/csrc/diffuse_bspline.hip
@@ -89,16 +89,17 @@
 template <int R, int T>
 __global__ __launch_bounds__(256) void bspline_decompose_strip(const float4 *__restrict__ in, float4 *__restrict__ hf,
                                                                float4 *__restrict__ lf, const int width, const int height,
-                                                               const int mult, const int groups, const int strip,
-                                                               const int strips_per_class, const unsigned *__restrict__ gate)
+                                                               const int mult, const int groups, const strip_plan_t plan,
+                                                               const unsigned *__restrict__ gate)
 {
   if(gate && *gate == 0u) return;
   __shared__ float4 vert[2][(T + 4) * R + 2];
   const int bx = blockIdx.x;
-  const int cls = blockIdx.y / strips_per_class, k0s = (blockIdx.y - cls * strips_per_class) * strip;
+  const strip_block_t sb = strip_of_block(plan, blockIdx.y);
+  const int cls = sb.cls, k0s = sb.k0;
   const int n_cls = (height - cls + mult - 1) / mult;
   if(k0s >= n_cls) return;
-  const int nrows = (strip < n_cls - k0s) ? strip : n_cls - k0s;
+  const int nrows = (sb.rows < n_cls - k0s) ? sb.rows : n_cls - k0s;
   const int r_first = cls + k0s * mult;
   const int group = bx % groups, tile = bx / groups;
   const int r0 = group * R, k0 = tile * T;
@@ -197,8 +198,8 @@
 }
 template <int R, int T, bool IN4>
 __global__ __launch_bounds__(256) void bspline_decompose_strip3(const void *__restrict__ in_v, bs_px3 *__restrict__ lf,
-                                                                const int width, const int height, const int strip,
-                                                                const int strips_per_class, unsigned *__restrict__ alpha_flag)
+                                                                const int width, const int height, const strip_plan_t plan,
+                                                                unsigned *__restrict__ alpha_flag)
 {
   static_assert(R * T == 256, "a workgroup's columns: one span of 256");
   constexpr int mult = R;
@@ -217,10 +218,11 @@
     else
       return in3[i];
   };
-  const int cls = blockIdx.y / strips_per_class, k0s = (blockIdx.y - cls * strips_per_class) * strip;
+  const strip_block_t sb = strip_of_block(plan, blockIdx.y);
+  const int cls = sb.cls, k0s = sb.k0;
   const int n_cls = (height - cls + mult - 1) / mult;
   if(k0s >= n_cls) return;
-  const int nrows = (strip < n_cls - k0s) ? strip : n_cls - k0s;
+  const int nrows = (sb.rows < n_cls - k0s) ? sb.rows : n_cls - k0s;
   const int r_first = cls + k0s * mult;
   const int k0 = (int)blockIdx.x * T;
   const int tid = threadIdx.x;
@@ -463,22 +465,23 @@
 
 int bspline_launch_decompose3(int devid, hipStream_t s, const void *in, bool in4, float *lf, int w, int h, int mult, unsigned *alpha_flag)
 {
-  (void)devid;
   if(mult != 1 && mult != 2 && mult != 4 && mult != 8 && mult != 16) return DT_HIP_INVALID_ARG;
   if(in4 && mult != 1) return DT_HIP_INVALID_ARG;
   const int classes = h < mult ? h : mult, per_class = (h + mult - 1) / mult;
   const int gx = (w + 255) / 256;
   const int strip = strip_rows(gx, classes, per_class);
-  const int spc = (per_class + strip - 1) / strip;
-  const dim3 grid(gx, classes * spc);
   launch_scope ls(devid, "diffuse_decompose");
   bs_px3 *const out = reinterpret_cast<bs_px3 *>(lf);
-  if(in4) bspline_decompose_strip3<1, 256, true><<<grid, 256, 0, s>>>(in, out, w, h, strip, spc, alpha_flag);
-  else if(mult == 1) bspline_decompose_strip3<1, 256, false><<<grid, 256, 0, s>>>(in, out, w, h, strip, spc, alpha_flag);
-  else if(mult == 2) bspline_decompose_strip3<2, 128, false><<<grid, 256, 0, s>>>(in, out, w, h, strip, spc, alpha_flag);
-  else if(mult == 4) bspline_decompose_strip3<4, 64, false><<<grid, 256, 0, s>>>(in, out, w, h, strip, spc, alpha_flag);
-  else if(mult == 8) bspline_decompose_strip3<8, 32, false><<<grid, 256, 0, s>>>(in, out, w, h, strip, spc, alpha_flag);
-  else bspline_decompose_strip3<16, 16, false><<<grid, 256, 0, s>>>(in, out, w, h, strip, spc, alpha_flag);
+  auto launch = [&](auto kernel) {
+    const strip_plan_t plan = strip_plan(gx, classes, per_class, strip, strip_resident(devid, (const void *)kernel, 0));
+    kernel<<<dim3(gx, strip_plan_blocks(plan, classes)), 256, 0, s>>>(in, out, w, h, plan, alpha_flag);
+  };
+  if(in4) launch(bspline_decompose_strip3<1, 256, true>);
+  else if(mult == 1) launch(bspline_decompose_strip3<1, 256, false>);
+  else if(mult == 2) launch(bspline_decompose_strip3<2, 128, false>);
+  else if(mult == 4) launch(bspline_decompose_strip3<4, 64, false>);
+  else if(mult == 8) launch(bspline_decompose_strip3<8, 32, false>);
+  else launch(bspline_decompose_strip3<16, 16, false>);
   return check_launch("diffuse_decompose");
 }
 
@@ -510,12 +513,14 @@
   const int classes = h < mult ? h : mult, per_class = (h + mult - 1) / mult;
   const int gx = mult == 1 ? (steps + 255) / 256 : (mult == 2 ? (steps + 127) / 128 : (mult == 4 ? (steps + 63) / 64 : ((steps + 31) / 32) * (mult / 8)));
   const int strip = strip_rows(gx, classes, per_class);
-  const int spc = (per_class + strip - 1) / strip;
-  const dim3 grid(gx, classes * spc);
-  if(mult == 1) bspline_decompose_strip<1, 256><<<grid, 256, 0, s>>>(in, hf, lf, w, h, mult, 1, strip, spc, gate);
-  else if(mult == 2) bspline_decompose_strip<2, 128><<<grid, 256, 0, s>>>(in, hf, lf, w, h, mult, 1, strip, spc, gate);
-  else if(mult == 4) bspline_decompose_strip<4, 64><<<grid, 256, 0, s>>>(in, hf, lf, w, h, mult, 1, strip, spc, gate);
-  else bspline_decompose_strip<8, 32><<<grid, 256, 0, s>>>(in, hf, lf, w, h, mult, mult / 8, strip, spc, gate);
+  auto launch = [&](auto kernel, const int groups) {
+    const strip_plan_t plan = strip_plan(gx, classes, per_class, strip, strip_resident(devid, (const void *)kernel, 0));
+    kernel<<<dim3(gx, strip_plan_blocks(plan, classes)), 256, 0, s>>>(in, hf, lf, w, h, mult, groups, plan, gate);
+  };
+  if(mult == 1) launch(bspline_decompose_strip<1, 256>, 1);
+  else if(mult == 2) launch(bspline_decompose_strip<2, 128>, 1);
+  else if(mult == 4) launch(bspline_decompose_strip<4, 64>, 1);
+  else launch(bspline_decompose_strip<8, 32>, mult / 8);
   return check_launch("diffuse_decompose");
 }
 }
diff --git a/ansel_amd/csrc/hip_common.h b/ansel_amd/csrc/hip_common.h
--- a/ansel_amd/csrc/hip_common.h
+++ b/ansel_amd/csrc/hip_common.h
@@ -25,6 +25,8 @@
   DISPATCH_AMAZE_BLOCKS,
   DISPATCH_BILAT_BLUR_SPLIT,
   DISPATCH_STRIP_ROWS,
+  DISPATCH_STRIP_TAIL,
+  DISPATCH_STRIP_TAIL_SHORT,
   DISPATCH_KEYS
 };
 int dispatch_override(dispatch_key_t key);
@@ -37,6 +39,69 @@
   while(strip > 4 && (size_t)gx * classes * ((per_class + strip - 1) / strip) < 2048) strip /= 2;
   return strip;
 }
+
+struct strip_plan_t
+{
+  int strip, spc;
+  int y_long;
+  int short_rows, q;
+};
+struct strip_block_t
+{
+  int cls, k0, rows;
+};
+constexpr int STRIP_TAIL_HALF_ROUNDS = 2, STRIP_TAIL_CUT = 4;
+static inline strip_plan_t strip_plan(const int gx, const int classes, const int per_class, const int strip, const int resident)
+{
+  strip_plan_t p;
+  p.strip = strip;
+  p.spc = (per_class + strip - 1) / strip;
+  const long long all = (long long)classes * p.spc;
+  const int forced = dispatch_override(DISPATCH_STRIP_TAIL), forced_cut = dispatch_override(DISPATCH_STRIP_TAIL_SHORT);
+  const int cut = forced > 0 && forced_cut ? forced_cut : STRIP_TAIL_CUT;
+  p.short_rows = (strip + cut - 1) / cut;
+  p.q = (strip + p.short_rows - 1) / p.short_rows;
+  long long y_tail = 0;
+  if(forced > 0)
+    y_tail = forced < all ? forced : all;
+  else if(forced == 0 && resident > 0 && p.q > 1 && (long long)gx * all >= 2ll * resident)
+  {
+    const long long per_tail = (long long)gx * p.q;
+    y_tail = ((long long)STRIP_TAIL_HALF_ROUNDS * resident + per_tail) / (2 * per_tail);
+    if(y_tail < 1) y_tail = 1;
+    if(y_tail > all) y_tail = all;
+    if(2 * y_tail * per_tail < resident || y_tail * per_tail > 2ll * resident) y_tail = 0;
+  }
+  if(y_tail == 0 || p.q == 1)
+  {
+    y_tail = 0;
+    p.short_rows = strip;
+    p.q = 1;
+  }
+  p.y_long = (int)(all - y_tail);
+  return p;
+}
+static inline unsigned strip_plan_blocks(const strip_plan_t &p, const int classes)
+{
+  return (unsigned)(p.y_long + (classes * p.spc - p.y_long) * p.q);
+}
+__host__ __device__ __forceinline__ strip_block_t strip_of_block(const strip_plan_t &p, const int by)
+{
+  int e = by, off = 0, rows = p.strip;
+  if(by >= p.y_long)
+  {
+    const int t = by - p.y_long, piece = t % p.q;
+    e = p.y_long + t / p.q;
+    off = piece * p.short_rows;
+    rows = p.short_rows < p.strip - off ? p.short_rows : p.strip - off;
+  }
+  strip_block_t b;
+  b.cls = e / p.spc;
+  b.k0 = (e - b.cls * p.spc) * p.strip + off;
+  b.rows = rows;
+  return b;
+}
+int strip_resident(int devid, const void *kernel, size_t lds);
 
 void set_last_error(const char *fmt, ...);
 
diff --git a/ansel_amd/csrc/runtime.cpp b/ansel_amd/csrc/runtime.cpp
--- a/ansel_amd/csrc/runtime.cpp
+++ b/ansel_amd/csrc/runtime.cpp
@@ -7,6 +7,7 @@
 #include <map>
 #include <vector>
 #include <string>
+#include <tuple>
 #include <stdarg.h>
 
 namespace
@@ -22,6 +23,7 @@
 {
   int hip_id = -1;
   std::string name;
+  int cus = 0;
   hipStream_t stream = nullptr;
   bool own_stream = false;
   std::mutex lock;
@@ -57,6 +59,8 @@
 std::vector<device_t *> g_devs;
 std::unordered_map<void *, alloc_t> g_allocs;
 thread_local char t_error[512] = "";
+std::mutex g_resident_lock;
+std::map<std::tuple<int, const void *, size_t>, int> g_resident;
 
 }
 
@@ -118,6 +122,22 @@
   }
   st.used = true;
   return DT_HIP_SUCCESS;
+}
+
+int strip_resident(int devid, const void *kernel, size_t lds)
+{
+  if(!make_current(devid) || !kernel) return 0;
+  std::lock_guard<std::mutex> g(g_resident_lock);
+  const auto key = std::make_tuple(devid, kernel, lds);
+  const auto it = g_resident.find(key);
+  if(it != g_resident.end()) return it->second;
+  int per_cu = 0;
+  if(hipOccupancyMaxActiveBlocksPerMultiprocessor(&per_cu, kernel, 256, lds) != hipSuccess || per_cu < 0)
+  {
+    (void)hipGetLastError();
+    per_cu = 0;
+  }
+  return g_resident[key] = per_cu * g_devs[devid]->cus;
 }
 
 hipStream_t stream_of(int devid)
@@ -196,6 +216,7 @@
     device_t *d = new device_t;
     d->hip_id = i;
     d->name = prop.name[0] ? prop.name : prop.gcnArchName;
+    d->cus = prop.multiProcessorCount;
     if(hipSetDevice(i) != hipSuccess || hipStreamCreateWithFlags(&d->stream, hipStreamNonBlocking) != hipSuccess)
     {
       delete d;
@@ -419,6 +440,27 @@
     }
   }
   return p;
+}
+
+int dt_hip_test_strip_residents(char *out, size_t cap)
+{
+  if(!out || cap < 1) return -1;
+  std::lock_guard<std::mutex> g(g_resident_lock);
+  size_t used = 0;
+  out[0] = 0;
+  for(const auto &kv : g_resident)
+  {
+    const int devid = std::get<0>(kv.first);
+    const char *const name = make_current(devid) ? hipKernelNameRefByPtr(std::get<1>(kv.first), g_devs[devid]->stream) : nullptr;
+    const int n = snprintf(out + used, cap - used, "%d %d %zu %s\n", devid, kv.second, std::get<2>(kv.first), name ? name : "?");
+    if(n < 0 || (size_t)n >= cap - used)
+    {
+      out[used] = 0;
+      continue;
+    }
+    used += (size_t)n;
+  }
+  return (int)g_resident.size();
 }
 
 int dt_hip_test_pool_fill(int devid, int enable, uint32_t pattern)
diff --git a/ansel_amd/csrc/testhooks.hip b/ansel_amd/csrc/testhooks.hip
--- a/ansel_amd/csrc/testhooks.hip
+++ b/ansel_amd/csrc/testhooks.hip
@@ -11,7 +11,7 @@
 {
 std::atomic<int> g_dispatch[DISPATCH_KEYS];
 const char *const g_dispatch_names[DISPATCH_KEYS] = { "nlm_v2", "nlm_fused", "amaze_unfused", "amaze_slab", "amaze_blocks",
-                                                       "bilat_blur_split", "strip_rows" };
+                                                       "bilat_blur_split", "strip_rows", "strip_tail", "strip_tail_short" };
 }
 namespace ansel
 {
@@ -24,6 +24,8 @@
     if(!strcmp(key, g_dispatch_names[k]))
     {
       if(k == DISPATCH_STRIP_ROWS && value != 0 && value != 4 && value != 8 && value != 16 && value != 32) return DT_HIP_INVALID_ARG;
+      if(k == DISPATCH_STRIP_TAIL && value < -1) return DT_HIP_INVALID_ARG;
+      if(k == DISPATCH_STRIP_TAIL_SHORT && value != 0 && value != 2 && value != 4 && value != 8) return DT_HIP_INVALID_ARG;
       g_dispatch[k].store(value);
       return DT_HIP_SUCCESS;
     }
@@ -31,6 +33,26 @@
 }
 
 extern "C" int dt_hip_test_strip_rows(int gx, int classes, int per_class) { return strip_rows(gx, classes, per_class); }
+extern "C" int dt_hip_test_strip_plan(int gx, int classes, int per_class, int strip, int resident, int *out)
+{
+  if(!out || gx < 1 || classes < 1 || per_class < 1 || strip < 1 || resident < 0) return DT_HIP_INVALID_ARG;
+  const strip_plan_t p = strip_plan(gx, classes, per_class, strip, resident);
+  const int v[6] = { p.strip, p.spc, p.y_long, p.short_rows, p.q, (int)strip_plan_blocks(p, classes) };
+  memcpy(out, v, sizeof(v));
+  return DT_HIP_SUCCESS;
+}
+extern "C" int dt_hip_test_strip_block(const int *plan, int by0, int n, int *out)
+{
+  if(!plan || !out || by0 < 0 || n < 0 || plan[0] < 1 || plan[1] < 1 || plan[2] < 0 || plan[3] < 1 || plan[4] < 1) return DT_HIP_INVALID_ARG;
+  strip_plan_t p;
+  p.strip = plan[0], p.spc = plan[1], p.y_long = plan[2], p.short_rows = plan[3], p.q = plan[4];
+  for(int k = 0; k < n; k++)
+  {
+    const strip_block_t b = strip_of_block(p, by0 + k);
+    out[3 * k] = b.cls, out[3 * k + 1] = b.k0, out[3 * k + 2] = b.rows;
+  }
+  return DT_HIP_SUCCESS;
+}
 
 namespace
 {
diff --git a/ansel_amd/lib.py b/ansel_amd/lib.py
--- a/ansel_amd/lib.py
+++ b/ansel_amd/lib.py
@@ -182,6 +182,9 @@
         "dt_hip_iop_highlights_resolve": (i, [i, vp, vp]),
         "dt_hip_test_dispatch": (i, [C.c_char_p, i]),
         "dt_hip_test_strip_rows": (i, [i, i, i]),
+        "dt_hip_test_strip_plan": (i, [i, i, i, i, i, P(i)]),
+        "dt_hip_test_strip_block": (i, [P(i), i, i, P(i)]),
+        "dt_hip_test_strip_residents": (i, [C.c_char_p, sz]),
         "dt_hip_test_nlm_last": (i, [P(i)]),
         "dt_hip_test_pool_fill": (i, [i, i, u]),
     }
@@ -208,6 +211,32 @@
     return load().dt_hip_test_strip_rows(int(gx), int(classes), int(per_class))
 
 
+STRIP_TAIL_ALL = 1 << 30
+
+
+def test_strip_plan(gx, classes, per_class, strip, resident):
+    out = (C.c_int * 6)()
+    check(load().dt_hip_test_strip_plan(int(gx), int(classes), int(per_class), int(strip), int(resident), out), "dt_hip_test_strip_plan")
+    return dict(zip(("strip", "spc", "y_long", "short_rows", "q", "blocks"), list(out)))
+
+
+def test_strip_blocks(plan, by0=0, n=None):
+    import numpy as np
+    n = plan["blocks"] - by0 if n is None else int(n)
+    p = (C.c_int * 5)(*[int(plan[k]) for k in ("strip", "spc", "y_long", "short_rows", "q")])
+    out = np.empty((n, 3), dtype=np.int32)
+    check(load().dt_hip_test_strip_block(p, int(by0), n, out.ctypes.data_as(C.POINTER(C.c_int))), "dt_hip_test_strip_block")
+    return out
+
+
+def test_strip_residents():
+    buf = C.create_string_buffer(1 << 16)
+    n = load().dt_hip_test_strip_residents(buf, len(buf))
+    rows = [ln.split(" ", 3) for ln in buf.value.decode().splitlines()]
+    assert n == len(rows), (n, len(rows))
+    return [(int(r[0]), int(r[1]), int(r[2]), r[3]) for r in rows]
+
+
 def test_pool_fill(devid, enable, pattern=0):
     was = load().dt_hip_test_pool_fill(devid, 1 if enable else 0, int(pattern) & 0xFFFFFFFF)
     if was < 0:
```
